# GregDMeyer/dynamite

Measured on AMD Instinct MI355X. Metric: matrix-free H|psi> Gamplitudes/s, random-field Heisenberg, higher is better.
Workload: dtype f64 (complex128)

## Files before the change

dynamite_amd/_lib.py:

```python
import ctypes as C
import os

import numpy as np

from . import build as _build

_HERE = os.path.dirname(os.path.abspath(__file__))

i64p = C.POINTER(C.c_int64)
f64p = C.POINTER(C.c_double)
vp = C.c_void_p


class Subspace(C.Structure):
    _fields_ = [("type", C.c_int32), ("L", C.c_int64), ("space", C.c_int64), ("k", C.c_int64),
                ("ld_nchoosek", C.c_int64), ("nchoosek", i64p), ("dim", C.c_int64),
                ("state_map", i64p), ("rmap_indices", i64p), ("rmap_states", i64p), ("vec_swizzle", C.c_int32),
                ("site_perm", C.POINTER(C.c_int8))]


class Partition(C.Structure):
    _fields_ = [("rank", C.c_int32), ("nranks", C.c_int32)]


MULT_FN = C.CFUNCTYPE(C.c_int, vp, vp, vp)
REDUCE_FN = C.CFUNCTYPE(C.c_int, vp, f64p, C.c_int)


class Hooks(C.Structure):
    _fields_ = [("ctx", vp), ("mult", MULT_FN), ("allreduce_sum", REDUCE_FN),
                ("allreduce_max", REDUCE_FN)]


class SolverStats(C.Structure):
    _fields_ = [("reason", C.c_int32), ("its", C.c_int32), ("matvecs", C.c_int32),
                ("nconv", C.c_int32), ("err_est", C.c_double)]


MAXSEG, MAXBSEG, MAXR = 4, 8, 16


LP_COUNT = 9
LP_NAMES = ["tile_real_k0", "tile_real", "tile_cplx", "tile_kvar_real", "tile_kvar_cplx", "gather_real",
            "gather_kvar_real", "gather_cplx", "gather_kvar_cplx"]
LP_KVAR, LP_CPLX, LP_GATHER = (3, 4, 6, 8), (2, 4, 7, 8), (5, 6, 7, 8)


class DevQuad(C.Structure):
    _fields_ = [("mask_tile", C.c_uint32), ("mask_loc", C.c_uint32), ("src", C.c_uint32),
                ("nslots", C.c_uint32), ("sign_tile", C.c_uint32 * 4), ("sign_ext", C.c_uint64 * 4),
                ("coeff", C.c_double * 4)]


class DevPass(C.Structure):
    _fields_ = [("nseg", C.c_int32), ("seg_off", C.c_int32 * MAXSEG), ("seg_len", C.c_int32 * MAXSEG),
                ("seg_pos", C.c_int32 * MAXSEG), ("nbseg", C.c_int32), ("bseg_off", C.c_int32 * MAXBSEG),
                ("bseg_len", C.c_int32 * MAXBSEG), ("bseg_pos", C.c_int32 * MAXBSEG),
                ("sign_base", C.c_uint64), ("accumulate", C.c_int32), ("need_tile", C.c_int32),
                ("has_diag", C.c_int32), ("cache_policy", C.c_int32), ("dext_begin", C.c_uint32), ("dext_end", C.c_uint32),
                ("dbucket", C.c_uint32 * (MAXR + 1)), ("loop", C.c_uint32 * (LP_COUNT + 1)),
                ("nquads", C.c_int32), ("n_eff", C.c_int32), ("quads", vp), ("dot_out", vp), ("zinit", vp), ("zscale", C.c_double), ("zinit2", vp), ("z2re", C.c_double), ("z2im", C.c_double),
                ("tile_bits", C.c_int32), ("log_rows", C.c_int32),
                ("swz_shift", C.c_int32), ("swz_xor_y", C.c_uint32), ("swz_xor_src", C.c_uint32), ("block_offset", C.c_uint32),
                ("pos_tmask", C.c_uint32), ("dtile", vp), ("tabs", vp), ("tabvals", vp), ("tab_loop", C.c_uint32 * 3),
                ("pad_tab", C.c_uint32), ("gbucket", C.c_uint32 * (MAXR + 1)), ("pad_g", C.c_uint32)]


class DevTab(C.Structure):
    _fields_ = [("mask_tile", C.c_uint32), ("mask_loc", C.c_uint32), ("src", C.c_uint32), ("first", C.c_uint32),
                ("z_tile", C.c_uint32), ("flags", C.c_uint32), ("tpos", C.c_uint32), ("twid", C.c_uint32),
                ("epos", C.c_uint32), ("ewid", C.c_uint32), ("z_ext", C.c_uint64), ("ik", C.c_uint64),
                ("ksign", C.c_uint32), ("nbits", C.c_uint32)]


class Xfer(C.Structure):
    _fields_ = [("partner", C.c_int32), ("pass_id", C.c_int32), ("offset", C.c_int64), ("count", C.c_int64)]


MAT_DEFAULT, MAT_FORCE_GATHER, MAT_USE_GLDS, MAT_HOST_ONLY = 0, 1, 2, 4
MAT_REAL_PACKED = 16
EXCHANGE_AUTO, EXCHANGE_PARTNER, EXCHANGE_TRANSPOSE = 0, 1, 2
PHASE_ALL, PHASE_EXCHANGE, PHASE_COMPUTE = 0, 1, 2
MAT_AMIN_SHIFT = 8
WHICH = {"lowest": 0, "highest": 1, "exterior": 2, "target": 3}
CONVERGED_TOL, CONVERGED_ITS, DIVERGED_ITS, DIVERGED_BREAKDOWN, DIVERGED_SYMMETRY_LOST = 1, 2, -1, -2, -3

SIGNATURES = {
    "dnm_last_error": (C.c_char_p, []),
    "dnm_version": (C.c_int, []),
    "dnm_device_count": (C.c_int, [C.POINTER(C.c_int)]),
    "dnm_set_device": (C.c_int, [C.c_int]),
    "dnm_malloc": (C.c_int, [C.POINTER(vp), C.c_size_t]),
    "dnm_free": (C.c_int, [vp]),
    "dnm_memcpy_h2d": (C.c_int, [vp, vp, C.c_size_t, vp]),
    "dnm_memcpy_d2h": (C.c_int, [vp, vp, C.c_size_t, vp]),
    "dnm_stream_synchronize": (C.c_int, [vp]),
    "dnm_subspace_dim": (C.c_int, [C.POINTER(Subspace), i64p]),
    "dnm_idx_to_state": (C.c_int, [C.POINTER(Subspace), C.c_int64, i64p, i64p]),
    "dnm_state_to_idx": (C.c_int, [C.POINTER(Subspace), C.c_int64, i64p, i64p]),
    "dnm_mat_create": (C.c_int, [C.c_int64, i64p, i64p, i64p, f64p, C.POINTER(Subspace),
                                 C.POINTER(Subspace), C.c_int, C.c_int, C.POINTER(Partition),
                                 C.POINTER(vp)]),
    "dnm_check_conserves": (C.c_int, [C.c_int64, i64p, i64p, i64p, f64p, C.POINTER(Subspace),
                                      C.POINTER(Subspace), C.c_int, C.POINTER(C.c_int), vp]),
    "dnm_reduced_density_matrix": (C.c_int, [vp, C.POINTER(Subspace), C.c_int, i64p, vp, vp]),
    "dnm_rdm_sector_plan": (C.c_int, [C.POINTER(Subspace), C.c_int, i64p, C.c_int, C.POINTER(C.c_int),
                                      C.POINTER(C.c_int32), i64p, i64p, C.POINTER(C.c_size_t)]),
    "dnm_rdm_sector_blocks": (C.c_int, [vp, C.POINTER(Subspace), C.c_int, i64p, C.c_int, C.c_int,
                                        C.POINTER(C.c_int32), C.POINTER(vp), vp]),
    "dnm_vec_set_random_swz": (C.c_int, [vp, C.c_int64, C.c_uint64, C.c_int64, C.c_int, vp]),
    "dnm_vec_swizzle_copy": (C.c_int, [vp, vp, C.c_int64, C.c_int, vp]),
    "dnm_vec_unpack_real": (C.c_int, [vp, vp, C.c_int64, C.c_int, C.c_int, vp]),
    "dnm_vec_layout_unpack_real": (C.c_int, [C.POINTER(Subspace), C.POINTER(Partition), vp, vp, vp]),
    "dnm_vec_layout_size": (C.c_int, [C.POINTER(Subspace), C.POINTER(C.c_int64)]),
    "dnm_vec_layout_partition": (C.c_int, [C.POINTER(Subspace), C.c_int, C.c_int, i64p, i64p, i64p, i64p]),
    "dnm_vec_layout_blocks": (C.c_int, [C.POINTER(Subspace), C.c_int64, i64p, i64p, i64p]),
    "dnm_vec_layout_copy": (C.c_int, [C.POINTER(Subspace), C.POINTER(Partition), vp, vp, C.c_int, vp]),
    "dnm_vec_layout_copy_f64": (C.c_int, [C.POINTER(Subspace), C.POINTER(Partition), vp, vp, C.c_int, vp]),
    "dnm_vec_layout_zero_padding": (C.c_int, [C.POINTER(Subspace), C.POINTER(Partition), vp, vp]),
    "dnm_vec_layout_positions": (C.c_int, [C.POINTER(Subspace), C.POINTER(Partition), C.c_int64, vp, vp, vp]),
    "dnm_vec_layout_positions_host": (C.c_int, [C.POINTER(Subspace), C.POINTER(Partition), C.c_int64, i64p, i64p]),
    "dnm_vec_layout_set_random": (C.c_int, [C.POINTER(Subspace), C.POINTER(Partition), vp, C.c_uint64, vp]),
    "dnm_mat_layouts": (C.c_int, [vp, C.POINTER(C.c_int), C.POINTER(C.c_int)]),
    "dnm_mat_window_split": (C.c_int, [vp, C.POINTER(C.c_int)]),
    "dnm_mat_mult_local_part": (C.c_int, [vp, vp, vp, C.c_int, C.c_int, vp]),
    "dnm_mat_local_part_bits": (C.c_int, [vp, C.POINTER(C.c_int), C.POINTER(C.c_int)]),
    "dnm_mat_mult_window_local": (C.c_int, [vp, vp, vp, vp]),
    "dnm_mat_mult_window_remote": (C.c_int, [vp, vp, C.c_int64, C.c_int64, vp, vp]),
    "dnm_mat_window_local_rows": (C.c_int, [vp, C.c_int64, C.c_int64, C.c_int, C.c_int, C.POINTER(C.c_int64), C.POINTER(C.c_int), vp]),
    "dnm_mat_mult_window_rows": (C.c_int, [vp, vp, C.c_int64, C.c_int64, vp, C.c_int64, C.c_int64, vp]),
    "dnm_mat_destroy": (C.c_int, [vp]),
    "dnm_mat_sizes": (C.c_int, [vp, i64p, i64p, i64p, i64p]),
    "dnm_mat_precompute_diagonal": (C.c_int, [vp, vp]),
    "dnm_mat_get_diagonal": (C.c_int, [vp, f64p, vp]),
    "dnm_mat_mult": (C.c_int, [vp, vp, vp, vp]),
    "dnm_mat_norm_inf": (C.c_int, [vp, f64p, vp]),
    "dnm_mat_set_norm": (C.c_int, [vp, C.c_double]),
    "dnm_mat_plan_describe": (C.c_int, [vp, C.c_char_p, C.c_size_t]),
    "dnm_mat_plan_launches": (C.c_int, [vp, C.POINTER(C.c_int)]),
    "dnm_mat_plan_counts": (C.c_int, [vp] + [C.POINTER(C.c_int)] * 6),
    "dnm_mat_export_dtile": (C.c_int, [vp, C.c_int, C.c_int, f64p, C.c_int64]),
    "dnm_mat_export_tabs": (C.c_int, [vp, C.c_int, C.c_int, vp, C.c_size_t, C.c_int, C.POINTER(C.c_int), f64p, C.c_int64, i64p]),
    "dnm_mat_export_pass": (C.c_int, [vp, C.c_int, C.c_int, vp, C.c_size_t, vp, C.c_size_t, C.c_int,
                                      C.POINTER(C.c_int)]),
    "dnm_mat_ownership": (C.c_int, [vp, i64p, i64p]),
    "dnm_mat_column_window": (C.c_int, [vp, i64p, i64p, vp]),
    "dnm_mat_column_chunks": (C.c_int, [vp, C.c_int, C.POINTER(C.c_uint8), C.c_int64, vp]),
    "dnm_mat_mult_window": (C.c_int, [vp, vp, C.c_int64, C.c_int64, vp, vp]),
    "dnm_mat_exchange_plan": (C.c_int, [vp, C.POINTER(C.c_int), C.POINTER(Xfer), C.POINTER(C.c_int),
                                        C.POINTER(Xfer)]),
    "dnm_mat_mult_dot": (C.c_int, [vp, vp, vp, f64p, vp]),
    "dnm_mat_mult_lanczos": (C.c_int, [vp, vp, vp, vp, C.c_double, f64p, vp]),
    "dnm_mat_mult_local": (C.c_int, [vp, vp, vp, vp]),
    "dnm_mat_mult_remote": (C.c_int, [vp, C.c_int32, vp, vp, vp]),
    "dnm_vec_set": (C.c_int, [vp, C.c_int64, C.c_double, C.c_double, vp]),
    "dnm_vec_copy": (C.c_int, [vp, vp, C.c_int64, vp]),
    "dnm_vec_scale": (C.c_int, [vp, C.c_int64, C.c_double, C.c_double, vp]),
    "dnm_vec_axpby": (C.c_int, [vp, vp, C.c_int64, C.c_double, C.c_double, C.c_double, C.c_double, vp]),
    "dnm_vec_dot": (C.c_int, [vp, vp, C.c_int64, f64p, vp]),
    "dnm_vec_norm2": (C.c_int, [vp, C.c_int64, f64p, vp]),
    "dnm_vec_set_random": (C.c_int, [vp, C.c_int64, C.c_uint64, C.c_int64, vp]),
    "dnm_vec_mdot": (C.c_int, [vp, C.c_int64, C.c_int, vp, C.c_int64, f64p, vp]),
    "dnm_vec_maxpy": (C.c_int, [vp, vp, C.c_int64, C.c_int, C.c_int64, f64p, vp]),
    "dnm_vec_basis_update": (C.c_int, [vp, C.c_int64, C.c_int, C.c_int, C.c_int64, f64p, vp]),
    "dnm_workspace_bytes": (C.c_int, [C.POINTER(C.c_size_t)]),
    "dnm_release_workspace": (C.c_int, []),
    "dnm_mat_is_real_packed": (C.c_int, [C.c_void_p, C.POINTER(C.c_int)]),
    "dnm_comm_unique_id": (C.c_int, [C.c_void_p]),
    "dnm_comm_create": (C.c_int, [C.c_void_p, C.c_int, C.c_int, C.POINTER(C.c_void_p)]),
    "dnm_comm_destroy": (C.c_int, [C.c_void_p]),
    "dnm_comm_forget": (C.c_int, [C.c_void_p, C.c_void_p]),
    "dnm_comm_loopback": (C.c_int, [C.c_void_p, C.c_int, C.c_int, C.POINTER(C.c_void_p), C.POINTER(C.c_void_p)]),
    "dnm_comm_allreduce": (C.c_int, [C.c_void_p, C.POINTER(C.c_double), C.c_int, C.c_int]),
    "dnm_mat_mult_partitioned": (C.c_int, [C.c_void_p, C.c_void_p, C.c_void_p, C.c_void_p, C.c_void_p]),
    "dnm_mat_column_ranges": (C.c_int, [C.c_void_p, C.c_int64, C.POINTER(C.c_int64), C.POINTER(C.c_int64)]),
    "dnm_comm_prepare": (C.c_int, [C.c_void_p, C.c_void_p, C.c_void_p]),
    "dnm_comm_set_phase": (C.c_int, [C.c_void_p, C.c_int]),
    "dnm_mat_set_exchange": (C.c_int, [C.c_void_p, C.c_int, C.POINTER(C.c_int)]),
    "dnm_mat_operator": (C.c_int, [C.c_void_p, i64p, i64p, i64p, i64p, i64p, f64p]),
    "dnm_mat_exchange_parts": (C.c_int, [C.c_void_p, C.POINTER(C.c_void_p), C.POINTER(C.c_void_p), C.POINTER(C.c_int)]),
    "dnm_comm_hooks": (C.c_int, [C.c_void_p, C.c_void_p, C.c_void_p, C.POINTER(Hooks)]),
    "dnm_sc_choose_site_perm": (C.c_int, [C.c_int, C.c_int, C.c_int, C.c_int64, i64p, C.c_int, C.POINTER(C.c_int8),
                                          C.POINTER(C.c_int32)]),
    "dnm_workspace_reserve": (C.c_int, [C.c_size_t, C.c_void_p]),
    "dnm_expm_chebyshev": (C.c_int, [vp, vp, vp, C.c_int64, C.c_double, C.c_double, C.POINTER(Hooks),
                                     C.POINTER(SolverStats), vp]),
    "dnm_mat_mult_sub": (C.c_int, [vp, vp, vp, vp, C.c_double, vp]),
    "dnm_mat_fuses_init": (C.c_int, [vp]),
    "dnm_mat_mult_sub2": (C.c_int, [vp, vp, vp, vp, C.c_double, vp, C.c_double, C.c_double, vp]),
    "dnm_expm_multiply": (C.c_int, [vp, vp, vp, C.c_int64, C.c_double, C.c_double, C.c_double, C.c_int,
                                    C.c_int, C.c_size_t, C.POINTER(Hooks), C.POINTER(SolverStats), vp]),
    "dnm_eigsolve": (C.c_int, [vp, C.c_int64, C.c_int, C.c_int, C.c_double, C.c_int, C.c_int,
                               C.c_uint64, C.POINTER(Hooks), C.c_int, f64p, vp,
                               C.POINTER(SolverStats), vp]),
    "dnm_eigsolve_interior": (C.c_int, [vp, C.c_int64, C.c_int, C.c_double, C.c_double, C.c_int, C.c_int,
                                        C.c_uint64, C.POINTER(Hooks), C.c_int, f64p, vp,
                                        C.POINTER(SolverStats), vp]),
    "dnm_interior_filter_plan": (C.c_int, [C.c_double, C.c_double, C.c_double, C.c_double, C.c_double,
                                           C.POINTER(C.c_int), f64p, f64p]),
}


class BackendError(RuntimeError):
    """Raised when a C-ABI call returns non-zero (the reference raises petsc4py.Error)."""


_lib = None


def lib():
    global _lib
    if _lib is None:
        import torch
        path = _build.build()
        import os
        if os.environ.get("DNM_EXPERIMENTAL") == "1":
            path = os.environ.get("DNM_LIB", path)
        L = C.CDLL(path)
        for name, (res, args) in SIGNATURES.items():
            fn = getattr(L, name)
            fn.restype = res
            fn.argtypes = args
        _lib = L
    return _lib


def check(rc):
    if rc != 0:
        raise BackendError(lib().dnm_last_error().decode())


def p64(a):
    return a.ctypes.data_as(i64p)


def pf64(a):
    return a.ctypes.data_as(f64p)


def device_count():
    n = C.c_int(0)
    lib().dnm_device_count(C.byref(n))
    return n.value
```

dynamite_amd/csrc/kernels.h:

```cpp
#pragma once

#include <vector>

#include "plan.h"
#include "subspace.h"

namespace dnm {

struct DevMsc {
  int32_t nmasks;
  const int64_t *masks;
  const int64_t *mask_offsets;
  const int64_t *signs;
  const double *real_coeffs;
};

bool tile_config_supported(int B, int logR);

int launch_tile_pass(const DevPass &P, int B, int logR, bool glds, int n_loc,
                     const void *x, void *y, const void *xr, hipStream_t st, unsigned nparts = 1);

struct ColMark {
  uint8_t *map = nullptr;
  int32_t shift = 0;
  int64_t first = 0;
};
int gather_num_blocks(int64_t M);
int gather_rows_per_block();
int launch_gather_matvec(const DevMsc &msc, const SubView &left, const SubView &right,
                         int64_t M, const double *diag, const void *x, void *y,
                         hipStream_t st, int64_t row0 = 0, int64_t win_start = 0, int xswz = -1,
                         int64_t *colrange = nullptr, ColMark mark = ColMark());

struct ScMask {
  int32_t fast;
  int32_t lo;
  double up_re, up_im, dn_re, dn_im;
  int32_t pair, hi, dead, pad;
};
std::vector<ScMask> sc_masks(const std::vector<int64_t> &masks, const std::vector<int64_t> &mask_offsets,
                             const std::vector<int64_t> &signs, const std::vector<double> &rcoef, int L = 0,
                             bool xparity = false);

struct ScLow {
  const uint16_t *tab;
  int32_t off[18];
};
int sc_num_blocks(int64_t M);
int sc_rows_per_block();
int launch_sc_matvec(const DevMsc &msc, const ScMask *scm, const ScLow &low, const SubView &sub, int64_t M, int64_t row0,
                     int64_t win_start, const double *diag, const void *xw, void *y, int64_t *colrange,
                     hipStream_t st, ColMark mark = ColMark());

struct ScBlock {
  const uint16_t *lowtab;
  int32_t off[18];
  int32_t lb;
  int32_t swizzle;
  int64_t h_first, h_last;
  const uint32_t *perm;
  int64_t nperm;
};
bool sc_block_supported(int lb);
int sc_block_max_masks();
int64_t sc_block_grid(const ScBlock &blk);
int launch_sc_block(const DevMsc &msc, const ScMask *scm, const ScBlock &blk, const SubView &sub, int64_t M, int64_t row0,
                    int64_t win_start, int64_t win_len, const double *diag, const void *xw, void *y,
                    hipStream_t st, const void *zinit = nullptr, double zscale = 0.0, double *dot_out = nullptr,
                    const void *zinit2 = nullptr, double z2re = 0.0, double z2im = 0.0);

int launch_diag(const DevMsc &msc, const SubView &sub, int64_t M, int64_t row0, double *diag, hipStream_t st);

int norm_num_blocks(int64_t M);
int launch_norm(const DevMsc &msc, const SubView &left, const SubView &right, int64_t M,
                int64_t row0, double *block_max, hipStream_t st);

int launch_conserves(const DevMsc &msc, const double *coeffs_im, const SubView &left, const SubView &right,
                     int64_t N, int *bad, hipStream_t st);

struct RdmGeom {
  int32_t k, L;
  int32_t nseg_keep, nseg_tr;
  int8_t klen[33], kpos[33];
  int8_t tlen[33], tpos[33];
};
void rdm_plan(const RdmGeom &geo, int *logtm, int *ntiles, int *nsplit, int64_t *chunks_per_split,
              size_t *partial_bytes);
int launch_rdm(const void *x, const SubView &sub, const RdmGeom &geo, void *partial, void *rho, hipStream_t st);
size_t rdm_partial_bytes(int64_t nsplit, int64_t nelem);
int rdm_sum_slices(void *partial, int64_t nelem, int *nsplit, void **level, hipStream_t st);

struct RdmSectorBlock {
  int32_t n, m;
  int64_t dim, traced;
  int64_t per_slice;
  void *out;
};
struct RdmSectorTile {
  int32_t blk, ti, tj, pad;
};
int rdm_sector_plan(int nblocks, RdmSectorBlock *blocks, int64_t *ntiles, int *nsplit, size_t *table_bytes,
                    size_t *partial_bytes);
int launch_rdm_sector(const void *x, const SubView &sub, const RdmGeom &geo, bool contig, int xparity_sector,
                      int nblocks, const RdmSectorBlock *blocks, int64_t ntiles, int nsplit, size_t table_bytes,
                      void *scratch, hipStream_t st);

int vk_set(void *x, int64_t n, double re, double im, hipStream_t st);
int vk_copy(void *y, const void *x, int64_t n, hipStream_t st);
int vk_scale(void *x, int64_t n, double re, double im, hipStream_t st);
int vk_axpby(void *y, const void *x, int64_t n, double are, double aim, double bre, double bim,
             hipStream_t st);
int vk_random(void *x, int64_t n, uint64_t seed, int64_t offset, hipStream_t st, int swz = 0);
int vk_swizzle_copy(void *dst, const void *src, int64_t n, int swz, hipStream_t st);
int vk_unpack_real(void *dst, const void *src, int64_t n_packed, int swz_src, int swz_dst, hipStream_t st);
int vk_mdot_blocks(int64_t n);
int vk_sweep_blocks(int64_t n);
size_t vk_sweep_scratch(int64_t n, int ncols);
int vk_mdot(const void *V, int64_t ldv, int nv, const void *w, int64_t n, double *partials_dev,
            hipStream_t st);
int vk_maxpy(void *w, const void *V, int64_t ldv, int nv, int64_t n, const double *c_dev,
             hipStream_t st);
int vk_basis_update(void *V, int64_t ldv, int nin, int nout, int64_t n, const double *S_dev,
                    hipStream_t st);
int vk_lanczos_update(void *p, const void *v, const void *u, int64_t n, double are, double aim, double b,
                      double scale, double *partials_dev, hipStream_t st);
int vk_lanczos_dot(void *y, const void *z, const void *x, int64_t n, double b, double *partials_dev,
                   hipStream_t st,
                   double yscale = 1.0);
size_t vk_reduce_scratch(int ncols);
int vk_reduce_partials(const double *partials, int nblocks, int ncols, double *out, hipStream_t st, double *tmp = nullptr);
int vk_norm2_partials(const void *x, int64_t n, double *partials_dev, hipStream_t st);

}
```

dynamite_amd/csrc/mat.cpp:

```cpp
#include "mat.h"
#include "vec_api.h"
#include "row_fused.h"

#include <algorithm>
#include <cstring>

namespace dnm {

static thread_local std::string g_err;

void set_error(const char *fmt, ...) {
  char buf[1024];
  va_list ap;
  va_start(ap, fmt);
  vsnprintf(buf, sizeof(buf), fmt, ap);
  va_end(ap);
  g_err = buf;
}

int DevBuf::alloc(size_t nbytes) {
  release();
  if (nbytes == 0) nbytes = 16;
  DNM_HIP(hipMalloc(&p, nbytes));
  bytes = nbytes;
// ... 75 lines not shown
      ++bucket[(size_t)(st >> host.bucket_shift) + 1];
    }
    if (sorted) {
      for (int64_t b = 0; b < nb; ++b) bucket[(size_t)b + 1] += bucket[(size_t)b];
      host.bucket = bucket.data();
    } else {
      bucket.clear();
      host.bucket = nullptr;
    }
  }
  host.dim = sub_dim(host);
  dev = host;
  dev.nchoosek = nullptr;
  dev.state_map = dev.rmap_indices = dev.rmap_states = nullptr;
  dev.bucket = nullptr;
  if (want_device) {
    if (!nck.empty()) {
      DNM_TRY(d_nck.upload(nck.data(), nck.size() * 8));
      dev.nchoosek = (const int64_t *)d_nck.p;
    }
    if (!smap.empty()) {
      DNM_TRY(d_smap.upload(smap.data(), smap.size() * 8));
      DNM_TRY(d_rstates.upload(rstates.data(), rstates.size() * 8));
      dev.state_map = (const int64_t *)d_smap.p;
      dev.rmap_states = (const int64_t *)d_rstates.p;
      if (!rind.empty()) {
        DNM_TRY(d_rind.upload(rind.data(), rind.size() * 8));
        dev.rmap_indices = (const int64_t *)d_rind.p;
      }
      if (!bucket.empty()) {
        DNM_TRY(d_bucket.upload(bucket.data(), bucket.size() * 8));
        dev.bucket = (const int64_t *)d_bucket.p;
      }
    }
  }
  return 0;
}

static int build_opform(const dnm_mat &A, OpForm *op) {
  const SubView &l = A.left.host, &r = A.right.host;
  const bool par = l.type == DNM_PARITY;
  const int n = par ? l.L - 1 : l.L;
  op->n = n;
  op->masks.clear();
  const uint64_t ones = n >= 64 ? ~0ull : (((uint64_t)1 << n) - 1);
  for (size_t mi = 0; mi < A.masks.size(); ++mi) {
    const uint64_t mask = (uint64_t)A.masks[mi];
    if (par && (parity64(mask) != (l.space ^ r.space))) continue;
    RowMask rm;
    rm.mask = par ? (mask >> 1) : mask;
    for (int64_t t = A.mask_offsets[mi]; t < A.mask_offsets[mi + 1]; ++t) {
      const uint64_t sg = (uint64_t)A.signs[t];
      RowTerm rt;
      rt.is_imag = parity64(mask & sg);
      double c = A.real_coeffs[t];
      uint64_t s2 = sg;
      if (par) {
        s2 = sg >> 1;
        if (sg & 1) {
          s2 ^= ones;
          if (r.space) c = -c;
        }
      }
      if (parity64(rm.mask & s2)) c = -c;
      rt.sign = s2;
      rt.coeff = c;
      rm.terms.push_back(rt);
    }
    if (rm.mask == 0) {
      RowMask im;
      im.mask = 0;
      im.zero_mask_offdiag = true;
      std::vector<RowTerm> re;
      for (const RowTerm &t : rm.terms) (t.is_imag ? im.terms : re).push_back(t);
      rm.terms.swap(re);
      if (!im.terms.empty()) op->masks.push_back(std::move(im));
      if (rm.terms.empty()) continue;
    }
    op->masks.push_back(std::move(rm));
  }
  std::stable_sort(op->masks.begin(), op->masks.end(),
            [](const RowMask &a, const RowMask &b) { return a.mask < b.mask; });
  return 0;
}

static uint32_t compress_to_tile(uint64_t bits, const PassSpec &ps) {
  uint32_t out = 0;
  int off = 0;
  for (int j = 0; j < ps.nseg; ++j) {
    uint64_t seg = (bits >> ps.seg_pos[j]) & (((uint64_t)1 << ps.seg_len[j]) - 1);
    out |= (uint32_t)seg << off;
    off += ps.seg_len[j];
  }
  return out;
}

static int pack_opform(OpForm *op) {
  DNM_CHECK(op->n >= 2, "real-packed form needs at least two index bits");
  std::vector<RowMask> out;
  for (const RowMask &rm : op->masks) {
    for (const RowTerm &t : rm.terms) DNM_CHECK(!t.is_imag, "operator has an imaginary matrix element: no real-packed form");
    DNM_CHECK(!rm.zero_mask_offdiag, "operator has an imaginary matrix element: no real-packed form");
    RowMask lanes;
    lanes.mask = rm.mask >> 1;
    lanes.pack_flip = (rm.mask & 1) != 0;
    if (rm.mask == 0) {
      RowMask diag;
      diag.mask = 0;
      lanes.zero_mask_offdiag = true;
      for (const RowTerm &t : rm.terms) {
        if (!(t.sign & 1)) { diag.terms.push_back({t.sign >> 1, t.coeff, 0}); continue; }
        lanes.terms.push_back({t.sign >> 1, t.coeff, 0});
        lanes.terms.push_back({t.sign >> 1, -t.coeff, 1});
      }
      if (!diag.terms.empty()) out.push_back(std::move(diag));
      if (!lanes.terms.empty()) out.push_back(std::move(lanes));
      continue;
    }
    lanes.zero_mask_offdiag = lanes.mask == 0;
    bool same = !lanes.pack_flip;
    for (const RowTerm &t : rm.terms) same = same && !(t.sign & 1);
    for (const RowTerm &t : rm.terms) {
      lanes.terms.push_back({t.sign >> 1, t.coeff, 0});
      if (!same) lanes.terms.push_back({t.sign >> 1, (t.sign & 1) ? -t.coeff : t.coeff, 1});
    }
    out.push_back(std::move(lanes));
  }
  std::stable_sort(out.begin(), out.end(), [](const RowMask &a, const RowMask &b) {
    if (a.mask != b.mask) return a.mask < b.mask;
    return (int)a.zero_mask_offdiag < (int)b.zero_mask_offdiag;
  });
  op->masks.swap(out);
  op->n -= 1;
  op->packed = true;
  return 0;
}

static bool table_form(const OpForm &op, const RowMask &m, std::vector<uint64_t> *zs) {
  const char *tabs_env = knob("DNM_TAB_RECORDS");
  if (tabs_env && tabs_env[0] == '0') return false;
  const int nb = __builtin_popcountll(m.mask);
  if (op.packed || m.pack_flip || nb < 1 || nb > MAXTABBITS || m.terms.size() < 5) return false;
  size_t nre = 0, nim = 0;
  zs->clear();
  for (const RowTerm &t : m.terms) {
    (t.is_imag ? nim : nre)++;
    const uint64_t z = t.sign & ~m.mask;
    if (std::find(zs->begin(), zs->end(), z) == zs->end()) zs->push_back(z);
  }
  const size_t nq = std::max((nre + 1) / 2, (nim + 1) / 2);
  return nq >= 2 && zs->size() * 45 < nq * 76;
}

static int build_pass(const dnm_mat &A, const PassSpec &ps, PassOnDevice *out) {
  const OpForm &op = A.op;
  const Plan &pl = A.plan;
  const int B = ps.B;
  int logR = ps.logR ? ps.logR : pl.cfg.logR;
  {
    std::vector<uint64_t> zs;
    bool any = false;
    for (int idx : ps.tile_masks) any = any || table_form(op, op.masks[idx], &zs);
    for (int idx : ps.gather_masks) any = any || table_form(op, op.masks[idx], &zs);
    int want = 3;
    if (const char *e = knob("DNM_TAB_LOG_ROWS")) want = atoi(e);
    if (any && want > logR && tile_config_supported(B, want)) logR = want;
  }
  {
    auto top_thread_pos = [&](int lr) {
      int c = 0, top = -1;
      for (int j = 0; j < ps.nseg; ++j)
        for (int i = 0; i < ps.seg_len[j]; ++i, ++c)
          if (c < B - lr) top = std::max(top, ps.seg_pos[j] + i);
      return top;
    };
    while (top_thread_pos(logR) >= 28 && tile_config_supported(B, logR + 1)) ++logR;
  }
  const int lognt = B - logR, R = 1 << logR;
  const int n_eff = ps.n_eff ? ps.n_eff : pl.n_loc;
  const uint64_t tb = ps.tile_bits();
  DevPass &d = out->desc;
  memset(&d, 0, sizeof(d));
  d.nseg = ps.nseg;
  int off = 0;
  for (int j = 0; j < ps.nseg; ++j) {
    d.seg_off[j] = off;
    d.seg_len[j] = ps.seg_len[j];
    d.seg_pos[j] = ps.seg_pos[j];
    off += ps.seg_len[j];
  }
  DNM_CHECK(off == B, "internal: tile segments do not add up to B");
  {
    std::vector<int> order;
    uint64_t gb = ps.glen ? ((((uint64_t)1 << ps.glen) - 1) << ps.gpos) : 0;
    std::vector<int> rest;
    for (int pos = 0; pos < n_eff; ++pos)
      if (!((tb >> pos) & 1) && !((gb >> pos) & 1)) rest.push_back(pos);
    size_t nsel = ps.glen ? std::min<size_t>(3, rest.size()) : 0;
    for (size_t i = 0; i < nsel; ++i) order.push_back(rest[i]);
    for (int pos = ps.gpos; pos < ps.gpos + ps.glen; ++pos) order.push_back(pos);
    for (size_t i = nsel; i < rest.size(); ++i) order.push_back(rest[i]);
    if (const char *e = knob("DNM_ORDER_WINDOW")) {
      if (ps.nseg > 1 && ps.partner < 0) {
        std::vector<int> o;
        for (const char *q = e; *q;) {
          o.push_back(atoi(q));
          while (*q && *q != ',') ++q;
          if (*q == ',') ++q;
        }
        std::vector<int> a = o, b2 = order;
        std::sort(a.begin(), a.end());
        std::sort(b2.begin(), b2.end());
        DNM_CHECK(a == b2, "DNM_ORDER_WINDOW is not a permutation of the block bits");
        order = o;
      }
    }
    DNM_CHECK((int)order.size() == n_eff - B, "internal: block bits do not add up");
    int nb = 0;
    for (size_t i = 0; i < order.size();) {
      size_t j = i + 1;
      while (j < order.size() && order[j] == order[j - 1] + 1) ++j;
      DNM_CHECK(nb < MAXBSEG, "internal: too many block segments");
      d.bseg_off[nb] = (int32_t)i;
      d.bseg_len[nb] = (int32_t)(j - i);
      d.bseg_pos[nb] = order[i];
      ++nb;
      i = j;
    }
    d.nbseg = nb;
  }
  d.sign_base = ((uint64_t)pl.rank << pl.n_loc) | ps.sign_extra;
  d.n_eff = n_eff;
  d.tile_bits = B;
  d.log_rows = logR;
  DNM_CHECK(tile_config_supported(B, logR), "unsupported tile configuration B=%d logR=%d", B, logR);
  d.accumulate = ps.accumulate ? 1 : 0;
  d.has_diag = 0;
  d.cache_policy = pl.cfg.cache_policy | (op.packed ? 256 : 0);
  {
    const int S = pl.cfg.swz;
    DNM_CHECK(S == 0 || (S >= 5 && S <= 24), "swizzle shift %d out of range", S);
    d.swz_shift = S;
    auto sw = [S](uint64_t v) -> uint32_t {
      return S ? (uint32_t)(((v >> S) & (((uint64_t)1 << (S - 4)) - 1)) << 4) : 0u;
    };
    d.swz_xor_y = sw((uint64_t)ps.y_off);
    d.swz_xor_src = sw((uint64_t)ps.src_off);
    uint64_t tm = 0;
    int c = 0;
    for (int j = 0; j < ps.nseg; ++j)
      for (int i = 0; i < ps.seg_len[j]; ++i, ++c)
        if (c < lognt) tm |= ((uint64_t)1 << (ps.seg_pos[j] + i)) | sw((uint64_t)1 << (ps.seg_pos[j] + i));
    DNM_CHECK((tm >> 28) == 0, "internal: thread bits of the tile above bit 27 (tile %llx, %d rows per thread)",
              (unsigned long long)tb, R);
    d.pos_tmask = (uint32_t)tm;
  }

  std::vector<DevQuad> quads;
  auto empty_quad = [&]() {
    DevQuad q;
    memset(&q, 0, sizeof(q));
    return q;
  };
  auto set_slot = [&](DevQuad &q, int slot, const RowTerm &t) {
    q.sign_ext[slot] = t.sign & ~tb;
    q.sign_tile[slot] = compress_to_tile(t.sign & tb, ps);
    q.coeff[slot] = t.coeff;
  };
  auto push_diag_list = [&](const std::vector<RowTerm> &lst) {
    for (size_t i = 0; i < lst.size(); i += 4) {
      DevQuad q = empty_quad();
      for (size_t j = i; j < lst.size() && j < i + 4; ++j) {
        set_slot(q, (int)(j - i), lst[j]);
        q.nslots = (uint32_t)(j - i + 1);
      }
      quads.push_back(q);
    }
  };

  if (ps.has_diag) {
    const RowMask *dm = nullptr;
    for (const RowMask &m : op.masks) if (m.mask == 0 && !m.zero_mask_offdiag) dm = &m;
    if (dm) {
      d.has_diag = 1;
      std::vector<RowTerm> lst;
      for (const RowTerm &t : dm->terms)
        if (compress_to_tile(t.sign & tb, ps) == 0) lst.push_back(t);
      d.dext_begin = (uint32_t)quads.size();
      push_diag_list(lst);
      d.dext_end = (uint32_t)quads.size();
      const char *dte = knob("DNM_DIAG_TABLE");
      const bool use_table = !(dte && dte[0] == '0') && B <= 13;
      if (use_table) out->h_dtile.assign((size_t)1 << B, 0.0);
      std::vector<std::pair<uint32_t, std::vector<RowTerm>>> groups;
      {
        const char *dge = knob("DNM_DIAG_GROUPS");
        const bool grouping = !(dge && dge[0] == '0') && !op.packed && !(A.flags & DNM_MAT_USE_GLDS);
        std::vector<std::pair<uint32_t, std::vector<RowTerm>>> all;
        if (grouping)
          for (const RowTerm &t : dm->terms) {
            const uint32_t st = compress_to_tile(t.sign & tb, ps);
            if (st == 0 || (t.sign & ~tb) == 0) continue;
            auto it = std::find_if(all.begin(), all.end(), [&](const auto &g) { return g.first == st; });
            if (it == all.end()) { all.push_back({st, {}}); it = all.end() - 1; }
            it->second.push_back(t);
          }
        std::stable_sort(all.begin(), all.end(), [](const auto &a, const auto &b) { return a.second.size() > b.second.size(); });
        for (auto &g : all)
          if (g.second.size() >= 3 && groups.size() < MAXDGROUPS) groups.push_back(std::move(g));
      }
      auto grouped = [&](uint32_t st) {
        return std::any_of(groups.begin(), groups.end(), [&](const auto &g) { return g.first == st; });
      };
      for (int j = 0; j < R; ++j) {
        lst.clear();
        for (const RowTerm &t : dm->terms) {
          uint32_t st = compress_to_tile(t.sign & tb, ps);
          if (st == 0 || (int)(st >> lognt) != j) continue;
          if (use_table && (t.sign & ~tb) == 0) {
            for (uint32_t tc = 0; tc < (1u << B); ++tc)
              out->h_dtile[tc] += (__builtin_popcount(tc & st) & 1) ? -t.coeff : t.coeff;
          } else if ((t.sign & ~tb) != 0 && grouped(st)) {
            continue;
          } else {
            lst.push_back(t);
          }
        }
        d.dbucket[j] = (uint32_t)quads.size();
        push_diag_list(lst);
      }
      for (int j = R; j <= MAXR; ++j) d.dbucket[j] = (uint32_t)quads.size();
      std::vector<std::pair<uint32_t, uint32_t>> where(groups.size());
      for (size_t g = 0; g < groups.size(); ++g) {
        std::vector<RowTerm> outside = groups[g].second;
        for (RowTerm &t : outside) t.sign &= ~tb;
        where[g].first = (uint32_t)quads.size();
        push_diag_list(outside);
        where[g].second = (uint32_t)quads.size() - where[g].first;
      }
      for (int j = 0; j < R; ++j) {
        d.gbucket[j] = (uint32_t)quads.size();
        for (size_t g = 0; g < groups.size(); ++g) {
          if ((int)(groups[g].first >> lognt) != j) continue;
          DevQuad q = empty_quad();
          q.sign_tile[0] = groups[g].first;
          q.mask_loc = where[g].first;
          q.src = where[g].second;
          q.nslots = 1;
          quads.push_back(q);
        }
      }
      for (int j = R; j <= MAXR; ++j) d.gbucket[j] = (uint32_t)quads.size();
    }
  }

  struct Rec { int loop; DevQuad q; };
  std::vector<Rec> recs;
  std::vector<DevTab> tabs_tile, tabs_gather;
  std::vector<double> tabvals;
  auto push_tabs = [&](const RowMask &m, uint64_t mloc, bool gather, int src) -> bool {
    std::vector<uint64_t> zs;
    if (!table_form(op, m, &zs)) return false;
    const int nb = __builtin_popcountll(m.mask);
    int pb[MAXTABBITS];
    for (int q = 0, pos = 0; pos < 64; ++pos)
      if ((m.mask >> pos) & 1ull) pb[q++] = pos;
    for (uint64_t z : zs) {
      DevTab T;
      memset(&T, 0, sizeof(T));
      T.mask_tile = compress_to_tile(mloc & tb, ps);
      T.mask_loc = (uint32_t)mloc;
      T.src = (uint32_t)src;
      T.nbits = (uint32_t)nb;
      const uint32_t zt = compress_to_tile(z & tb, ps);
      T.z_tile = zt & ((1u << lognt) - 1u);
      T.z_ext = z & ~tb;
      T.first = (uint32_t)(tabvals.size() / 2);
      for (int k = 0; k < R; ++k)
        if (__builtin_popcount((uint32_t)k & (zt >> lognt)) & 1) T.ksign |= 1u << k;
      for (int q = 0; q < nb; ++q) {
        if ((tb >> pb[q]) & 1ull) {
          const int tpos = __builtin_ctz(compress_to_tile((uint64_t)1 << pb[q], ps));
          if (tpos < lognt) {
            T.tpos |= (uint32_t)tpos << (8 * q);
            T.twid |= 1u << (8 * q);
          } else {
            T.flags |= 1u;
            for (int k = 0; k < R; ++k)
              if ((k >> (tpos - lognt)) & 1) T.ik |= (uint64_t)1 << (4 * k + q);
          }
        } else {
          T.epos |= (uint32_t)pb[q] << (8 * q);
          T.ewid |= 1u << (8 * q);
        }
      }
      for (int j = 0; j < (1 << nb); ++j) {
        uint64_t rowbits = 0;
        for (int q = 0; q < nb; ++q)
          if ((j >> q) & 1) rowbits |= (uint64_t)1 << pb[q];
        double re = 0.0, im = 0.0;
        for (const RowTerm &t : m.terms) {
          if ((t.sign & ~m.mask) != z) continue;
          const double c = (__builtin_popcountll(rowbits & t.sign & m.mask) & 1) ? -t.coeff : t.coeff;
          (t.is_imag ? im : re) += c;
        }
        tabvals.push_back(re);
        tabvals.push_back(im);
      }
      if (z == zs.back()) T.flags |= 2u;
      (gather ? tabs_gather : tabs_tile).push_back(T);
    }
    return true;
  };
  auto push_mask = [&](int idx, bool gather, int src) {
    const RowMask &m = op.masks[idx];
    const uint64_t mloc = m.mask & (((uint64_t)1 << n_eff) - 1);
    if (!gather) DNM_CHECK((mloc & ~tb) == 0, "internal: tile mask leaves the tile");
    if (push_tabs(m, mloc, gather, src)) return 0;
    std::vector<const RowTerm *> re, im;
    for (const RowTerm &t : m.terms) (t.is_imag ? im : re).push_back(&t);
    size_t ir = 0, ii = 0;
    while (ir < re.size() || ii < im.size()) {
      DevQuad q = empty_quad();
      q.mask_tile = compress_to_tile(mloc & tb, ps);
      q.mask_loc = (uint32_t)mloc;
      q.src = (uint32_t)src;
      q.nslots = m.pack_flip ? 1u : 0u;
      bool kvar = false, cplx = false;
      for (int s = 0; s < 2 && ir < re.size(); ++s, ++ir) {
        set_slot(q, s, *re[ir]);
        kvar |= (q.sign_tile[s] >> lognt) != 0;
      }
      for (int s = 2; s < 4 && ii < im.size(); ++s, ++ii) {
        set_slot(q, s, *im[ii]);
        kvar |= (q.sign_tile[s] >> lognt) != 0;
        cplx = true;
      }
      int loop;
      if (gather) loop = kvar ? (cplx ? LP_GATHER_KVAR_CPLX : LP_GATHER_KVAR_REAL) : (cplx ? LP_GATHER_CPLX : LP_GATHER_REAL);
      else if (kvar) loop = cplx ? LP_TILE_KVAR_CPLX : LP_TILE_KVAR_REAL;
      else if (cplx) loop = LP_TILE_CPLX;
      else loop = (q.mask_tile >> lognt) == 0 ? LP_TILE_REAL_K0 : LP_TILE_REAL;
      recs.push_back({loop, q});
    }
    return 0;
  };
  for (int idx : ps.tile_masks) DNM_TRY(push_mask(idx, false, 0));
  for (size_t i = 0; i < ps.gather_masks.size(); ++i)
    DNM_TRY(push_mask(ps.gather_masks[i], true, ps.gather_src[i]));
  for (int lp = 0; lp < LP_COUNT; ++lp) {
    d.loop[lp] = (uint32_t)quads.size();
    for (const Rec &r : recs) if (r.loop == lp) quads.push_back(r.q);
  }
  d.loop[LP_COUNT] = (uint32_t)quads.size();

  d.nquads = (int32_t)quads.size();
  d.need_tile = (d.has_diag || !ps.tile_masks.empty()) ? 1 : 0;
  d.tab_loop[0] = 0;
  d.tab_loop[1] = (uint32_t)tabs_tile.size();
  d.tab_loop[2] = (uint32_t)(tabs_tile.size() + tabs_gather.size());
  out->h_tabs = tabs_tile;
  out->h_tabs.insert(out->h_tabs.end(), tabs_gather.begin(), tabs_gather.end());
  out->h_tabvals = tabvals;
  d.tabs = nullptr;
  d.tabvals = nullptr;
  if (!out->h_tabs.empty() && !A.host_only) {
    DNM_TRY(out->tabs.upload(out->h_tabs.data(), out->h_tabs.size() * sizeof(DevTab)));
    DNM_TRY(out->tabvals.upload(out->h_tabvals.data(), out->h_tabvals.size() * sizeof(double)));
    d.tabs = (const DevTab *)out->tabs.p;
    d.tabvals = (const double *)out->tabvals.p;
  }
  out->h_quads = quads;
  if (!A.host_only) DNM_TRY(out->quads.upload(quads.data(), quads.size() * sizeof(DevQuad)));
  d.quads = (const DevQuad *)out->quads.p;
  d.dtile = nullptr;
  if (!out->h_dtile.empty() && !A.host_only) {
    DNM_TRY(out->dtile.upload(out->h_dtile.data(), out->h_dtile.size() * sizeof(double)));
    d.dtile = (const double *)out->dtile.p;
  }
  out->partner = ps.partner;
  out->n_eff = n_eff;
  out->y_off = ps.y_off;
  out->src_off = ps.src_off;
  return 0;
}

static hipStream_t S(void *stream) { return (hipStream_t)stream; }

static int launch_pass(const dnm_mat *A, const PassOnDevice &p, const DevPass &d, const void *x, void *y,
                       const void *xr, hipStream_t st, unsigned nparts = 1) {
  return launch_tile_pass(d, d.tile_bits, d.log_rows, (A->flags & DNM_MAT_USE_GLDS) != 0, p.n_eff, x, y, xr, st, nparts);
}

static size_t pass_dot_partials(const dnm_mat *, const PassOnDevice &p) {
  return (size_t)1 << (p.n_eff - p.desc.tile_bits);
}

}

using namespace dnm;

namespace dnm {
std::vector<ScMask> sc_masks(const std::vector<int64_t> &masks, const std::vector<int64_t> &mask_offsets,
                             const std::vector<int64_t> &signs, const std::vector<double> &rcoef, int L, bool xparity) {
  std::vector<ScMask> scm(masks.size());
  for (size_t mi = 0; mi < masks.size(); ++mi) {
    ScMask &e = scm[mi];
    memset(&e, 0, sizeof(e));
    const uint64_t mask = (uint64_t)masks[mi];
    e.dead = __builtin_popcountll(mask) & 1;
    if (xparity && L >= 3 && __builtin_popcountll(mask) == L - 2 && !((mask >> (L - 1)) & 1ull)) {
      const uint64_t miss = ~mask & ((((uint64_t)1 << (L - 1)) - 1));
      const int i = __builtin_ctzll(miss);
      const uint64_t pairbits = ((uint64_t)1 << i) | ((uint64_t)1 << (L - 1));
      bool local = true;
      for (int64_t t = mask_offsets[mi]; t < mask_offsets[mi + 1]; ++t)
        if ((uint64_t)signs[t] & ~pairbits) local = false;
      if (!local) continue;
      e.pair = 2;
      e.lo = i;
      e.hi = L - 1;
      for (int64_t t = mask_offsets[mi]; t < mask_offsets[mi + 1]; ++t) {
        const double c = (((uint64_t)signs[t] >> i) & 1) ? -rcoef[t] : rcoef[t];
        e.up_re += c;
        e.dn_re += c;
      }
      continue;
    }
    if (__builtin_popcountll(mask) != 2) continue;
    const int lo = __builtin_ctzll(mask), hi = 63 - __builtin_clzll(mask);
    bool local = true;
    for (int64_t t = mask_offsets[mi]; t < mask_offsets[mi + 1]; ++t)
      if ((uint64_t)signs[t] & ~mask) local = false;
    if (!local) continue;
    e.pair = 1;
    e.fast = hi == lo + 1;
    e.lo = lo;
    e.hi = hi;
    for (int64_t t = mask_offsets[mi]; t < mask_offsets[mi + 1]; ++t) {
      const uint64_t sg = (uint64_t)signs[t];
      const double rc = rcoef[t];
      const bool imag = parity64(mask & sg);
      const double up = ((sg >> hi) & 1) ? -rc : rc;
      const double dn = ((sg >> lo) & 1) ? -rc : rc;
      (imag ? e.up_im : e.up_re) += up;
      (imag ? e.dn_im : e.dn_re) += dn;
    }
  }
  return scm;
}
}

extern "C" {

const char *dnm_last_error(void) { return g_err.c_str(); }
int dnm_version(void) { return 100; }

int dnm_device_count(int *count) {
  DNM_CHECK(count, "null pointer");
  hipError_t e = hipGetDeviceCount(count);
  if (e != hipSuccess) { *count = 0; (void)hipGetLastError(); }
  return 0;
}
int dnm_set_device(int device) { DNM_HIP(hipSetDevice(device)); return 0; }
int dnm_malloc(void **dptr, size_t bytes) { DNM_HIP(hipMalloc(dptr, bytes ? bytes : 16)); return 0; }
int dnm_free(void *dptr) { DNM_HIP(hipFree(dptr)); return 0; }
int dnm_memcpy_h2d(void *dst, const void *src, size_t bytes, void *stream) {
  DNM_HIP(hipMemcpyAsync(dst, src, bytes, hipMemcpyHostToDevice, S(stream)));
  DNM_HIP(hipStreamSynchronize(S(stream)));
  return 0;
}
int dnm_memcpy_d2h(void *dst, const void *src, size_t bytes, void *stream) {
  DNM_HIP(hipMemcpyAsync(dst, src, bytes, hipMemcpyDeviceToHost, S(stream)));
  DNM_HIP(hipStreamSynchronize(S(stream)));
  return 0;
}
int dnm_stream_synchronize(void *stream) { DNM_HIP(hipStreamSynchronize(S(stream))); return 0; }

int dnm_subspace_dim(const dnm_subspace *s, int64_t *dim) {
  SubView v{};
  DNM_TRY(view_from_c(s, &v));
  *dim = sub_dim(v);
  return 0;
}

int dnm_idx_to_state(const dnm_subspace *s, int64_t n, const int64_t *idxs, int64_t *states) {
  SubView v{};
  DNM_TRY(view_from_c(s, &v));
  const int64_t dim = sub_dim(v);
  for (int64_t i = 0; i < n; ++i) {
    DNM_CHECK(idxs[i] >= 0 && idxs[i] < dim, "index %lld out of bounds for subspace of dimension %lld",
              (long long)idxs[i], (long long)dim);
    states[i] = sub_i2s(idxs[i], v);
  }
  return 0;
}

int dnm_state_to_idx(const dnm_subspace *s, int64_t n, const int64_t *states, int64_t *idxs) {
  SubView v{};
  DNM_TRY(view_from_c(s, &v));
  for (int64_t i = 0; i < n; ++i) idxs[i] = sub_s2i(states[i], v);
  return 0;
}

int dnm_check_conserves(int64_t nmasks, const int64_t *masks, const int64_t *mask_offsets,
                        const int64_t *signs, const double *coeffs, const dnm_subspace *left,
                        const dnm_subspace *right, int xparity, int *result, void *stream) {
  DNM_CHECK(result && (nmasks == 0 || (masks && mask_offsets && signs && coeffs)), "null argument");
  SubOwned l, r;
  DNM_TRY(l.init(left, true));
  DNM_TRY(r.init(right, true));
  const int64_t nterms = nmasks ? mask_offsets[nmasks] : 0;
  std::vector<double> re(nterms), im(nterms);
  for (int64_t t = 0; t < nterms; ++t) { re[t] = coeffs[2 * t]; im[t] = coeffs[2 * t + 1]; }
  DevBuf dm, doff, ds, dre, dim_, dbad;
  DNM_TRY(dm.upload(masks, (size_t)nmasks * 8));
  DNM_TRY(doff.upload(mask_offsets, (size_t)(nmasks + 1) * 8));
  DNM_TRY(ds.upload(signs, (size_t)nterms * 8));
  DNM_TRY(dre.upload(re.data(), (size_t)nterms * 8));
  DNM_TRY(dim_.upload(im.data(), (size_t)nterms * 8));
  int zero = 0;
  DNM_TRY(dbad.upload(&zero, sizeof(int)));
  DevMsc msc{(int32_t)nmasks, (const int64_t *)dm.p, (const int64_t *)doff.p, (const int64_t *)ds.p,
             (const double *)dre.p};
  const int64_t ncols = xparity ? r.host.dim / 2 : r.host.dim;
  DNM_TRY(launch_conserves(msc, (const double *)dim_.p, l.dev, r.dev, ncols, (int *)dbad.p, S(stream)));
  int bad = 0;
  DNM_TRY(dnm_memcpy_d2h(&bad, dbad.p, sizeof(int), stream));
  *result = bad ? 0 : 1;
  return 0;
}

static DevBuf g_rdm_scratch;
}
namespace dnm {
int rdm_release_scratch() {
  g_rdm_scratch.release();
  return 0;
}
}
extern "C" {

static void rdm_geom(int L, int keep_size, const int64_t *keep, RdmGeom *out) {
  RdmGeom &geo = *out;
// ... 304 lines not shown
  if (lt == DNM_SPIN_CONSERVE && rt == DNM_SPIN_CONSERVE)
    scm = sc_masks(A->masks, A->mask_offsets, A->signs, A->real_coeffs, A->left.host.L, A->xparity);
  if (!A->host_only) {
  DNM_TRY(A->d_masks.upload(A->masks.data(), A->masks.size() * 8));
  DNM_TRY(A->d_offsets.upload(A->mask_offsets.data(), A->mask_offsets.size() * 8));
  DNM_TRY(A->d_signs.upload(A->signs.data(), A->signs.size() * 8));
  DNM_TRY(A->d_rcoeffs.upload(A->real_coeffs.data(), A->real_coeffs.size() * 8));
  A->dmsc.nmasks = (int32_t)nmasks;
  A->dmsc.masks = (const int64_t *)A->d_masks.p;
  A->dmsc.mask_offsets = (const int64_t *)A->d_offsets.p;
  A->dmsc.signs = (const int64_t *)A->d_signs.p;
  A->dmsc.real_coeffs = (const double *)A->d_rcoeffs.p;
  if (lt == DNM_SPIN_CONSERVE && rt == DNM_SPIN_CONSERVE) {
    A->sc_nfast = 0;
    for (const ScMask &e : scm) A->sc_nfast += e.fast ? 1 : 0;
    DNM_TRY(A->d_scmasks.upload(scm.data(), scm.size() * sizeof(ScMask)));
    std::vector<uint16_t> low(65536);
    int cnt[18] = {0};
    for (int v = 0; v < 65536; ++v) ++cnt[__builtin_popcount(v) + 1];
    for (int j = 0; j < 17; ++j) { cnt[j + 1] += cnt[j]; A->sclow.off[j] = cnt[j]; }
    A->sclow.off[17] = 65536;
    int fill[17];
    for (int j = 0; j < 17; ++j) fill[j] = A->sclow.off[j];
    for (int v = 0; v < 65536; ++v) low[fill[__builtin_popcount(v)]++] = (uint16_t)v;
    DNM_TRY(A->d_sclow.upload(low.data(), low.size() * sizeof(uint16_t)));
    A->sclow.tab = (const uint16_t *)A->d_sclow.p;
    if (!A->use_sc3) DNM_TRY(setup_sc_block(A.get()));
  }
  }
  if (A->use_sc3) {
    const SubView &h = A->left.host;
    const Sc3Layout *ly = sc3_get(h.L, h.k, sc3_code_a(h.sc3), sc3_code_w(h.sc3), !A->host_only, sc3_code_order(h.sc3));
    DNM_CHECK(ly, "could not build the SpinConserve vector layout");
    A->sc3.reset(new Sc3Mat());
    std::vector<uint32_t> Tb = sc3_partition(*ly, A->nranks);
    if (A->xparity) Tb = {0u, 1u << (ly->host.t - 1)};
    const bool want_real = (flags & DNM_MAT_REAL_PACKED) != 0;
    Sc3Perm P, Pr;
    DNM_CHECK(sc3_perm_make(left->site_perm, h.L, &P) && sc3_perm_make(right->site_perm, h.L, &Pr),
              "site_perm is not a permutation of the %d spins", h.L);
    DNM_CHECK(memcmp(P.to_int, Pr.to_int, sizeof P.to_int) == 0, "left and right vectors must share their site relabelling");
    DNM_CHECK(!P.on || A->nranks == 1, "a relabelled SpinConserve layout is not partitioned over ranks");
    DNM_CHECK(!A->xparity || P.to_int[h.L - 1] == h.L - 1, "XParity: the site relabelling must keep spin L-1 in place");
    A->sc3->perm = P;
    std::vector<int64_t> pmasks = A->masks, poffs = A->mask_offsets, psigns = A->signs;
    std::vector<double> pcoef = A->real_coeffs;
    if (P.on) {
      std::vector<int64_t> order((size_t)nmasks);
      std::vector<uint64_t> nm((size_t)nmasks);
      for (int64_t i = 0; i < nmasks; ++i) {
        order[(size_t)i] = i;
        nm[(size_t)i] = sc3_permute((uint64_t)A->masks[(size_t)i], P.to_int, h.L);
      }
      std::sort(order.begin(), order.end(), [&](int64_t x, int64_t y) { return nm[(size_t)x] < nm[(size_t)y]; });
      pmasks.clear(); psigns.clear(); pcoef.clear();
      poffs.assign(1, 0);
      for (int64_t q = 0; q < nmasks; ++q) {
        const int64_t i = order[(size_t)q];
        pmasks.push_back((int64_t)nm[(size_t)i]);
        for (int64_t t = A->mask_offsets[(size_t)i]; t < A->mask_offsets[(size_t)i + 1]; ++t) {
          psigns.push_back((int64_t)sc3_permute((uint64_t)A->signs[(size_t)t], P.to_int, h.L));
          pcoef.push_back(A->real_coeffs[(size_t)t]);
        }
        poffs.push_back((int64_t)psigns.size());
      }
      scm = sc_masks(pmasks, poffs, psigns, pcoef, h.L, A->xparity);
      if (!A->host_only) {
        DNM_TRY(A->d_pmasks.upload(pmasks.data(), pmasks.size() * 8));
        DNM_TRY(A->d_poffsets.upload(poffs.data(), poffs.size() * 8));
        DNM_TRY(A->d_psigns.upload(psigns.data(), psigns.size() * 8));
        DNM_TRY(A->d_prcoeffs.upload(pcoef.data(), pcoef.size() * 8));
      }
    }
    A->dmsc_sc3 = A->dmsc;
    if (P.on && !A->host_only) {
      A->dmsc_sc3.masks = (const int64_t *)A->d_pmasks.p;
      A->dmsc_sc3.mask_offsets = (const int64_t *)A->d_poffsets.p;
      A->dmsc_sc3.signs = (const int64_t *)A->d_psigns.p;
      A->dmsc_sc3.real_coeffs = (const double *)A->d_prcoeffs.p;
    }
    DNM_TRY(A->sc3->init(ly, pmasks, poffs, psigns, pcoef, scm, !A->host_only, Tb[A->rank],
                         Tb[A->rank + 1], want_real));
    if (const char *e = knob("DNM_SC3_TILED")) if (e[0] == '0') A->sc3->tiled = false;
    if (const char *e = knob("DNM_SC3_DIAG")) if (e[0] == 'c' && A->sc3->diag_mode == 2) A->sc3->diag_mode = 1;
    if (const char *e = knob("DNM_SC3_DIAG")) if (e[0] == 'n') A->sc3->diag_mode = 0;
    int64_t is, il, ns, nl;
    sc3_range(*ly, Tb[A->rank], Tb[A->rank + 1], &is, &il, &ns, &nl);
    A->m_local = A->n_local = il;
    A->rows_local = nl;
    A->row0 = ns;
    if (want_real) {
      DNM_CHECK(A->sc3->tiled && A->sc3->sym,
                "operator has an imaginary matrix element or is not a sum of pair hops: no real-packed form in this layout");
      A->real_packed = true;
      A->m_local = A->n_local = il / 2;
    }
  } else if (flags & DNM_MAT_REAL_PACKED) {
    DNM_CHECK(A->hypercube, "real-packed operators: Full / Parity pairs, or a SpinConserve pair in the internal layout");
  }

  if (A->hypercube) {
    DNM_TRY(build_opform(*A, &A->op));
    if (flags & DNM_MAT_REAL_PACKED) {
      DNM_CHECK(A->M == A->N, "real-packed operators: square");
      DNM_TRY(pack_opform(&A->op));
      A->real_packed = true;
      A->M /= 2; A->N /= 2; A->m_local /= 2; A->n_local /= 2;
    }
    if (A->xparity) {
      const uint64_t topbit = (uint64_t)1 << (A->op.n - 1);
      for (RowMask &rm : A->op.masks) {
        DNM_CHECK(!(rm.mask & topbit), "internal: XParity mask reaches the top index bit");
        for (RowTerm &t : rm.terms) t.sign &= ~topbit;
      }
      A->op.n -= 1;
    }
    PlanConfig cfg = plan_config_from_env();
    if (const int fa = (flags >> DNM_MAT_AMIN_SHIFT) & 0xff) cfg.amin = fa;
    DNM_CHECK(A->left.host.swz == A->right.host.swz, "left and right vectors of a Full/Parity pair must share a layout");
    cfg.swz = A->left.host.swz;
    if (cfg.logR < 0) {
      int nl = A->op.n;
      for (int r = A->nranks; r > 1; r >>= 1) --nl;
      cfg.logR = cfg.swz ? 2 : (nl >= 26 ? 4 : 3);
    }
    if (cfg.diag_last < 0) cfg.diag_last = cfg.swz ? 1 : 0;
    if (cfg.window_first < 0) {
      int nl = A->op.n;
      for (int r = A->nranks; r > 1; r >>= 1) --nl;
      cfg.window_first = (cfg.swz && nl >= 25) ? 1 : 0;
    }
    if (!tile_config_supported(cfg.B, cfg.logR)) {
      set_error("unsupported tile configuration B=%d logR=%d", cfg.B, cfg.logR);
      return 1;
    }
    DNM_TRY(make_plan(A->op, A->rank, A->nranks, cfg, &A->plan));
    if (flags & DNM_MAT_FORCE_GATHER) A->plan.use_tiled = false;
    DNM_CHECK(!A->real_packed || A->plan.use_tiled, "real-packed operators run on the tiled kernel only (vector too small)");
    if (A->nranks > 1 && !A->plan.use_tiled) {
      A->plan.remote.clear();
      A->plan.sends.clear();
    }
    if (A->plan.use_tiled) {
      for (const PassSpec &ps : A->plan.local) {
        std::unique_ptr<PassOnDevice> p(new PassOnDevice());
        DNM_TRY(build_pass(*A, ps, p.get()));
        A->local_passes.push_back(std::move(p));
      }
      for (const PassSpec &ps : A->plan.remote) {
        std::unique_ptr<PassOnDevice> p(new PassOnDevice());
        DNM_TRY(build_pass(*A, ps, p.get()));
        A->remote_passes.push_back(std::move(p));
      }
    }
  }
  *out = A.release();
  return 0;
}

int dnm_mat_destroy(dnm_mat *A) {
  delete A;
  return 0;
}

int dnm_mat_set_exchange(dnm_mat *A, int scheme, int *chosen) {
  DNM_CHECK(A && chosen, "null argument");
  DNM_CHECK(scheme == DNM_EXCHANGE_AUTO || scheme == DNM_EXCHANGE_PARTNER || scheme == DNM_EXCHANGE_TRANSPOSE,
            "unknown exchange scheme %d", scheme);
  delete A->tr_lo; delete A->tr_hi;
  A->tr_lo = A->tr_hi = nullptr;
  A->tr_f = -1;
  *chosen = DNM_EXCHANGE_PARTNER;
  const int P = A->nranks;
  if (scheme == DNM_EXCHANGE_PARTNER || P < 2 || (scheme == DNM_EXCHANGE_AUTO && P < 4)) return 0;
  const SubView &lh = A->left.host, &rh = A->right.host;
  if (!(A->hypercube && A->plan.use_tiled && !A->xparity && lh.type == rh.type && lh.L == rh.L &&
        (lh.type == DNM_FULL || lh.space == rh.space) && lh.swz == rh.swz))
    return 0;
  int p = 0;
  while ((1 << p) < P) ++p;
  const int shift = lh.type == DNM_PARITY ? 1 : 0;
  const int packed = A->real_packed ? 1 : 0;
  const int n = (int)lh.L - shift - p, f = n - 1 - p;
  if ((1 << p) != P || f < packed) return 0;
  if (lh.swz && f - packed < 2 * lh.swz - 4) return 0;
  const int fs = f + shift, ns = n + shift;
  const int64_t fld = P - 1;
  struct Term { int64_t m, s; double c; };
  std::vector<Term> lo, hi;
  for (size_t i = 0; i < A->masks.size(); ++i)
    for (int64_t t = A->mask_offsets[i]; t < A->mask_offsets[i + 1]; ++t) {
      const int64_t m = A->masks[i], s = A->signs[(size_t)t];
      if ((m >> ns) == 0) { lo.push_back({m, s, A->real_coeffs[(size_t)t]}); continue; }
      if ((m >> fs) & fld) return 0;
      auto swap = [&](int64_t v) {
        const int64_t d = ((v >> fs) ^ (v >> ns)) & fld;
        return v ^ (d << fs) ^ (d << ns);
      };
      hi.push_back({swap(m), swap(s), A->real_coeffs[(size_t)t]});
    }
  if (lo.empty() || hi.empty()) return 0;
  const int np = n - packed, fp = f - packed;
  dnm_subspace ld{}, rd{};
  ld.type = lh.type; ld.L = lh.L; ld.space = lh.space; ld.vec_swizzle = lh.swz;
  rd.type = rh.type; rd.L = rh.L; rd.space = rh.space; rd.vec_swizzle = rh.swz;
  const dnm_partition part{A->rank, A->nranks};
  dnm_mat *made[2] = {nullptr, nullptr};
  for (int which = 0; which < 2; ++which) {
    std::vector<Term> &T = which ? hi : lo;
    std::stable_sort(T.begin(), T.end(), [](const Term &a, const Term &b) { return a.m < b.m; });
    std::vector<int64_t> masks, offs, signs;
    std::vector<double> coeffs;
    for (size_t i = 0; i < T.size(); ++i) {
      if (i == 0 || T[i].m != T[i - 1].m) { masks.push_back(T[i].m); offs.push_back((int64_t)i); }
      signs.push_back(T[i].s);
      coeffs.push_back(T[i].c); coeffs.push_back(0.0);
    }
    offs.push_back((int64_t)T.size());
    int fl = A->flags & ~(0xff << DNM_MAT_AMIN_SHIFT);
    if (which == 1 && np - fp <= 8) {
      const char *tb = knob("DNM_TILE_BITS");
      const int a = (tb ? atoi(tb) : 12) - (np - fp);
      if (a >= 2 && a <= 9) fl |= a << DNM_MAT_AMIN_SHIFT;
    } else {
      fl |= A->flags & (0xff << DNM_MAT_AMIN_SHIFT);
    }
    int rc = dnm_mat_create((int64_t)masks.size(), masks.data(), offs.data(), signs.data(), coeffs.data(), &ld, &rd, 0, fl,
                            &part, &made[which]);
    int ns_ = 0, nr_ = 0;
    if (rc == 0) rc = dnm_mat_exchange_plan(made[which], &ns_, nullptr, &nr_, nullptr);
    if (rc == 0 && (ns_ || nr_)) { set_error("transposed exchange: a pass is not rank-local"); rc = 1; }
    if (rc == 0 && !(made[which]->hypercube && made[which]->plan.use_tiled)) {
      set_error("transposed exchange: a part of the operator has no tiled plan"); rc = 1;
    }
    if (rc != 0) { delete made[0]; delete made[1]; return rc; }
  }
  A->tr_lo = made[0];
  A->tr_hi = made[1];
  A->tr_f = fp;
  *chosen = DNM_EXCHANGE_TRANSPOSE;
  return 0;
}

int dnm_mat_operator(const dnm_mat *A, int64_t *nmasks, int64_t *nterms, int64_t *masks, int64_t *mask_offsets,
                     int64_t *signs, double *coeffs) {
  DNM_CHECK(A && nmasks && nterms, "null argument");
  *nmasks = (int64_t)A->masks.size();
  *nterms = (int64_t)A->signs.size();
  if (masks) std::copy(A->masks.begin(), A->masks.end(), masks);
  if (mask_offsets) std::copy(A->mask_offsets.begin(), A->mask_offsets.end(), mask_offsets);
  if (signs) std::copy(A->signs.begin(), A->signs.end(), signs);
  if (coeffs) std::copy(A->real_coeffs.begin(), A->real_coeffs.end(), coeffs);
  return 0;
}

int dnm_mat_exchange_parts(const dnm_mat *A, dnm_mat **lo, dnm_mat **hi, int *f) {
  DNM_CHECK(A && lo && hi && f, "null argument");
  *lo = A->tr_lo; *hi = A->tr_hi; *f = A->tr_f;
  return 0;
}

int dnm_mat_sizes(const dnm_mat *A, int64_t *M, int64_t *N, int64_t *m_local, int64_t *n_local) {
  DNM_CHECK(A, "null matrix");
  if (M) *M = A->M;
  if (N) *N = A->N;
  if (m_local) *m_local = A->m_local;
  if (n_local) *n_local = A->n_local;
  return 0;
}

int dnm_mat_layouts(const dnm_mat *A, int *left, int *right) {
  DNM_CHECK(A, "null matrix");
  if (left) *left = A->use_sc3 ? A->left.host.sc3 : A->left.host.swz;
  if (right) *right = A->use_sc3 ? A->right.host.sc3 : A->right.host.swz;
  return 0;
}

int dnm_mat_is_real_packed(const dnm_mat *A, int *packed) {
  DNM_CHECK(A && packed, "null argument");
  *packed = A->real_packed ? 1 : 0;
  return 0;
}

static int sc3_mult(dnm_mat *A, const void *x, void *y, const void *z, double b, const void *z2, double c_re, double c_im,
                    double *dot3_host, void *stream, int64_t win_start = -1, int phase = 0) {
  Sc3Call call;
  call.row0 = A->sc3->row0;
  call.win_start = win_start >= 0 ? win_start : A->sc3->row0;
  call.zinit = (const double2 *)z;
  call.zscale = b;
  call.zinit2 = (const double2 *)z2;
  call.z2re = c_re;
  call.z2im = c_im;
  const double *dg = A->have_diag ? (const double *)A->diag.p : nullptr;
  if (!dot3_host) return launch_sc3(*A->sc3, A->dmsc_sc3, call, dg, x, y, S(stream), phase);
  const size_t nwg = sc3_dot_partials(*A->sc3);
  double *part = nullptr;
  DNM_TRY(vec_scratch(((nwg + 1) * 3 + vk_reduce_scratch(3)) * sizeof(double), &part));
  call.dot_out = part;
  DNM_TRY(launch_sc3(*A->sc3, A->dmsc_sc3, call, dg, x, y, S(stream)));
  DNM_TRY(vk_reduce_partials(part, (int)nwg, 3, part + 3 * nwg, S(stream), part + 3 * nwg + 3));
  DNM_HIP(hipMemcpyAsync(dot3_host, part + 3 * nwg, 3 * sizeof(double), hipMemcpyDeviceToHost, S(stream)));
  DNM_HIP(hipStreamSynchronize(S(stream)));
  return 0;
}

// ... 430 lines not shown
  DNM_CHECK(A->use_sc3 && A->sc3->tiled, "this operator's window multiply does not split (dnm_mat_window_split)");
  int64_t lo, hi;
  DNM_TRY(dnm_mat_column_window(A, &lo, &hi, stream));
  DNM_CHECK(win_start <= lo && win_start + win_len > hi,
            "window [%lld, %lld) does not cover the positions [%lld, %lld] this rank reads", (long long)win_start,
            (long long)(win_start + win_len), (long long)lo, (long long)hi);
  return sc3_mult(A, x_window, y_local, nullptr, 0.0, nullptr, 0.0, 0.0, nullptr, stream,
                  A->real_packed ? 2 * win_start : win_start, 2);
}

int dnm_mat_exchange_plan(const dnm_mat *A, int *nsend, dnm_xfer *sends, int *nrecv, dnm_xfer *recvs) {
  DNM_CHECK(A && nsend && nrecv, "null argument");
  *nsend = (int)A->plan.sends.size();
  *nrecv = (int)A->remote_passes.size();
  if (sends)
    for (size_t i = 0; i < A->plan.sends.size(); ++i)
      sends[i] = {A->plan.sends[i].partner, -1, A->plan.sends[i].offset, A->plan.sends[i].count};
  if (recvs)
    for (size_t i = 0; i < A->remote_passes.size(); ++i) {
      const auto &p = A->remote_passes[i];
      recvs[i] = {p->partner, (int32_t)i, p->src_off, (int64_t)1 << p->n_eff};
    }
  return 0;
}

int dnm_mat_mult_remote(dnm_mat *A, int32_t recv_index, const void *x_recv, void *y, void *stream) {
  DNM_CHECK(A && x_recv && y, "null argument");
  DNM_CHECK(!A->host_only, "host-only handle cannot multiply");
  DNM_CHECK(recv_index >= 0 && recv_index < (int)A->remote_passes.size(), "rank %d has no receive %d", A->rank,
            recv_index);
  const auto &p = A->remote_passes[recv_index];
  return launch_pass(A, *p, p->desc, x_recv, (char *)y + (size_t)p->y_off * 16, x_recv, S(stream));
}

int dnm_mat_norm_inf(dnm_mat *A, double *nrm, void *stream) {
  DNM_CHECK(A && nrm, "null argument");
  DNM_CHECK(!A->host_only, "host-only handle has no device tables");
  if (A->nrm != -1.0) {
    *nrm = A->nrm;
    return 0;
  }
  const int nb = norm_num_blocks(A->rows_local);
  DNM_TRY(A->scratch.alloc((size_t)nb * sizeof(double)));
  DNM_TRY(launch_norm(A->dmsc, A->left.dev, A->right.dev, A->rows_local, A->row0,
                      (double *)A->scratch.p, S(stream)));
  std::vector<double> h(nb);
  DNM_TRY(dnm_memcpy_d2h(h.data(), A->scratch.p, (size_t)nb * sizeof(double), stream));
  double best = 0.0;
  for (double v : h) best = std::max(best, v);
  if (A->nranks == 1) A->nrm = best;
  *nrm = best;
  return 0;
}

int dnm_mat_set_norm(dnm_mat *A, double nrm) {
  DNM_CHECK(A, "null matrix");
  A->nrm = nrm;
  return 0;
}

int dnm_mat_plan_describe(const dnm_mat *A, char *buf, size_t buflen) {
  DNM_CHECK(A && buf && buflen, "null argument");
  std::string s;
  if (A->hypercube) s = A->plan.describe(A->op);
  else if (A->use_sc3) {
    const Sc3Tab &T = A->sc3->ly->host;
    char tmp[512];
    if (A->sc3->tiled && A->sc3->graph)
      snprintf(tmp, sizeof tmp, "SpinConserve two-pass kernels on a bond graph, internal layout [T %d | W %d | Lo %d]: "
               "window pass (%zu workgroups, %d hops in LDS, %d gathered) then lo pass (%zu workgroups, %d hops in LDS, "
               "%d gathered), diagonal %s, coefficients %s\n", T.t, T.w, T.a, A->sc3->permB.size(), A->sc3->op.nldsB,
               A->sc3->op.ngatB, A->sc3->permA.size() / 8, A->sc3->op.nldsA, A->sc3->op.ngatA,
               A->sc3->diag_mode == 2 ? "on the fly" : (A->sc3->diag_mode == 1 ? "cached" : "none"),
               A->sc3->sym ? "real symmetric" : "complex");
    else if (A->sc3->tiled)
      snprintf(tmp, sizeof tmp, "SpinConserve two-pass kernels, internal layout [T %d | W %d | Lo %d]: window pass (%zu "
               "workgroups, %d bonds in LDS, %d gathered) then lo pass (%zu workgroups, %d bonds in LDS, %d gathered), "
               "diagonal %s, coefficients %s\n", T.t, T.w, T.a, A->sc3->permB.size(), T.w - 1,
               __builtin_popcountll(A->sc3->op.bondsB), A->sc3->permA.size() / 8, T.a - 1,
               __builtin_popcountll(A->sc3->op.bondsA),
               A->sc3->diag_mode == 2 ? "on the fly" : (A->sc3->diag_mode == 1 ? "cached" : "none"),
               A->sc3->sym ? "real symmetric" : "complex");
    else
      snprintf(tmp, sizeof tmp, "SpinConserve row kernel, internal layout [T %d | W %d | Lo %d] (positions by table)\n",
               T.t, T.w, T.a);
    s = tmp;
  } else if (A->sc_pair)
    s = A->scblock.lb ? "SpinConserve kernel, block form (" + std::to_string(A->scblock.lb) +
                            " low bits per workgroup in LDS, high bonds as block runs)\n"
                      : std::string("SpinConserve kernel (one row per thread, incremental colex rank)\n");
  else s = A->nranks > 1 ? "generic row-gather kernel (rows split in index order, columns through a window)\n"
                         : "generic row-gather kernel (non-hypercube subspace pair)\n";
  if (A->hypercube && !A->plan.use_tiled) s += "generic row-gather kernel in use\n";
  if (A->hypercube && A->plan.use_tiled) {
    size_t ntab = 0, nquad = 0;
    for (const auto &p : A->local_passes) { ntab += p->h_tabs.size(); nquad += p->desc.loop[LP_COUNT] - p->desc.loop[0]; }
    for (const auto &p : A->remote_passes) { ntab += p->h_tabs.size(); nquad += p->desc.loop[LP_COUNT] - p->desc.loop[0]; }
    if (ntab) s += "table records: " + std::to_string(ntab) + " (beside " + std::to_string(nquad) + " records of four terms)\n";
  }
  snprintf(buf, buflen, "%s", s.c_str());
  return 0;
}

int dnm_mat_export_pass(const dnm_mat *A, int remote, int idx, void *desc_out, size_t desc_bytes,
                        void *quads_out, size_t quad_bytes, int max_quads, int *nquads) {
  DNM_CHECK(A && nquads, "null argument");
  const auto &v = remote ? A->remote_passes : A->local_passes;
  DNM_CHECK(idx >= 0 && idx < (int)v.size(), "pass index out of range");
  const PassOnDevice &p = *v[idx];
  *nquads = (int)p.h_quads.size();
  if (desc_out) {
    DNM_CHECK(desc_bytes == sizeof(DevPass), "DevPass size mismatch (%zu vs %zu)", desc_bytes, sizeof(DevPass));
    memcpy(desc_out, &p.desc, sizeof(DevPass));
  }
  if (quads_out) {
    DNM_CHECK(quad_bytes == sizeof(DevQuad), "DevQuad size mismatch (%zu vs %zu)", quad_bytes, sizeof(DevQuad));
    DNM_CHECK(max_quads >= *nquads, "record buffer too small");
    if (!p.h_quads.empty()) memcpy(quads_out, p.h_quads.data(), p.h_quads.size() * sizeof(DevQuad));
  }
  return 0;
}

int dnm_mat_export_tabs(const dnm_mat *A, int remote, int idx, void *tabs_out, size_t tab_bytes, int max_tabs, int *ntabs,
                        double *vals_out, int64_t max_vals, int64_t *nvals) {
  DNM_CHECK(A && ntabs && nvals, "null argument");
  const auto &v = remote ? A->remote_passes : A->local_passes;
  DNM_CHECK(idx >= 0 && idx < (int)v.size(), "pass index out of range");
  const PassOnDevice &p = *v[idx];
  *ntabs = (int)p.h_tabs.size();
  *nvals = (int64_t)p.h_tabvals.size();
  if (tabs_out && !p.h_tabs.empty()) {
    DNM_CHECK(tab_bytes == sizeof(DevTab), "DevTab size mismatch (%zu vs %zu)", tab_bytes, sizeof(DevTab));
    DNM_CHECK(max_tabs >= *ntabs, "record buffer too small");
    memcpy(tabs_out, p.h_tabs.data(), p.h_tabs.size() * sizeof(DevTab));
  }
  if (vals_out && !p.h_tabvals.empty()) {
    DNM_CHECK(max_vals >= *nvals, "table buffer too small");
    memcpy(vals_out, p.h_tabvals.data(), p.h_tabvals.size() * sizeof(double));
  }
  return 0;
}

int dnm_mat_export_dtile(const dnm_mat *A, int remote, int idx, double *out, int64_t n) {
  DNM_CHECK(A && out, "null argument");
  const auto &v = remote ? A->remote_passes : A->local_passes;
  DNM_CHECK(idx >= 0 && idx < (int)v.size(), "pass index out of range");
  const PassOnDevice &p = *v[idx];
  DNM_CHECK((int64_t)p.h_dtile.size() == n, "the pass has %zu tabulated diagonal entries, not %lld", p.h_dtile.size(),
            (long long)n);
  memcpy(out, p.h_dtile.data(), p.h_dtile.size() * sizeof(double));
  return 0;
}

int dnm_mat_plan_counts(const dnm_mat *A, int *n_local_passes, int *n_remote_passes, int *tiled,
                        int *B, int *logR, int *n_loc) {
  DNM_CHECK(A, "null matrix");
  if (n_local_passes) *n_local_passes = (int)A->local_passes.size();
  if (n_remote_passes) *n_remote_passes = (int)A->remote_passes.size();
  if (tiled) *tiled = (A->hypercube && A->plan.use_tiled) ? 1 : 0;
  if (B) *B = A->plan.cfg.B;
  if (logR) *logR = A->plan.cfg.logR;
  if (n_loc) *n_loc = A->plan.n_loc;
  return 0;
}

int dnm_mat_plan_launches(const dnm_mat *A, int *n) {
  DNM_CHECK(A && n, "null argument");
  *n = (A->hypercube && A->plan.use_tiled) ? (int)A->local_passes.size() : 1;
  return 0;
}

}

dnm_mat::~dnm_mat() {
  delete tr_lo;
  delete tr_hi;
}
```

dynamite_amd/csrc/mat.h:

```cpp
#pragma once

#include <memory>
#include <vector>

#include "kernels.h"
#include "plan.h"
#include "sc3.h"
#include "subspace.h"

namespace dnm {

struct DevBuf {
  void *p = nullptr;
  size_t bytes = 0;
  DevBuf() = default;
  DevBuf(const DevBuf &) = delete;
  DevBuf &operator=(const DevBuf &) = delete;
  ~DevBuf() { release(); }
  int alloc(size_t nbytes);
  int upload(const void *host, size_t nbytes);
  void release();
};

struct SubOwned {
  SubView host{};
  SubView dev{};
  std::vector<int64_t> nck, smap, rind, rstates, bucket;
  DevBuf d_nck, d_smap, d_rind, d_rstates, d_bucket;
  int init(const dnm_subspace *s, bool want_device);
};

struct PassOnDevice {
  DevPass desc{};
  std::vector<DevQuad> h_quads;
  DevBuf quads;
  std::vector<double> h_dtile;
  DevBuf dtile;
  std::vector<DevTab> h_tabs;
  std::vector<double> h_tabvals;
  DevBuf tabs, tabvals;
  int partner = -1;
  int n_eff = 0;
  int64_t y_off = 0, src_off = 0;
};

int rdm_release_scratch();

}

struct dnm_mat {
  std::vector<int64_t> masks, mask_offsets, signs;
  std::vector<double> real_coeffs;
  dnm::SubOwned left, right;
  int64_t M = 0, N = 0, m_local = 0, n_local = 0;
  int64_t row0 = 0;
  bool sc_pair = false;
  bool use_sc3 = false;
  std::unique_ptr<dnm::Sc3Mat> sc3;
  int64_t rows_local = 0;
  int64_t win_min = 0, win_max = -1;
  int rank = 0, nranks = 1;
  int flags = 0;
  bool xparity = false;
  bool host_only = false;

  bool hypercube = false;
  bool real_packed = false;
  dnm::OpForm op;
  dnm::Plan plan;
  std::vector<std::unique_ptr<dnm::PassOnDevice>> local_passes, remote_passes;

  dnm::DevBuf d_masks, d_offsets, d_signs, d_rcoeffs;
  dnm::DevMsc dmsc{};
  dnm::DevBuf d_pmasks, d_poffsets, d_psigns, d_prcoeffs;
  dnm::DevMsc dmsc_sc3{};
  dnm::DevBuf d_sclow;
  dnm::ScLow sclow{};
  dnm::DevBuf d_scblock;
  dnm::DevBuf d_scperm;
  dnm::ScBlock scblock{};
  bool row_fuse = true;
  int sc_nfast = 0;
  double expm_tstep = 0.0;
  int expm_m = 0;
  int expm_bound = 0;
  dnm::DevBuf d_scmasks;

  dnm_mat *tr_lo = nullptr, *tr_hi = nullptr;
  int tr_f = -1;
  ~dnm_mat();

  dnm::DevBuf diag;
  bool have_diag = false;
  double nrm = -1.0;
  dnm::DevBuf scratch;
};
```

dynamite_amd/csrc/matvec_kernels.hip:

```cpp
#include <algorithm>
#include <cstdint>
#include <cstdlib>

#include "kernels.h"

namespace dnm {

typedef double2 c128;

#define GLOBAL_AS __attribute__((address_space(1)))
#define LDS_AS __attribute__((address_space(3)))

typedef double d2v __attribute__((ext_vector_type(2)));

typedef const __attribute__((address_space(4))) DevQuad CQuad;

__device__ __forceinline__ void store_through(c128 *p, double re, double im) {
  d2v v = {re, im};
  asm volatile("global_store_dwordx4 %0, %1, off sc1\n\ts_nop 1" ::"v"(p), "v"(v) : "memory");
}
__device__ __forceinline__ void store_streaming(c128 *p, double re, double im) {
  d2v v = {re, im};
  __builtin_nontemporal_store(v, reinterpret_cast<d2v *>(p));
}
__device__ __forceinline__ c128 load_streaming(const c128 *p) {
  d2v v = __builtin_nontemporal_load(reinterpret_cast<const d2v *>(p));
  return make_double2(v.x, v.y);
}

#ifdef DNM_PHASE_TIMING
__device__ unsigned long long *g_phase_buf = nullptr;
#define DNM_PH(i, waitvm)                                                                                  \
  do {                                                                                                     \
    if (waitvm) asm volatile("s_waitcnt vmcnt(0)" ::: "memory");                                           \
    if (g_phase_buf && threadIdx.x == 0)                                                                   \
      g_phase_buf[((size_t)(P.accumulate ? gridDim.x : 0) + blockIdx.x) * 8 + (i)] = wall_clock64();        \
    asm volatile("" ::: "memory");                                                                         \
  } while (0)
#else
#define DNM_PH(i, waitvm)
#endif

#ifndef DNM_XP_PRIO
#define DNM_XP_PRIO 1
#endif
#if DNM_XP_PRIO == 1
#define DNM_PRIO_MEM() asm volatile("s_setprio 3")
#define DNM_PRIO_LDS() asm volatile("s_setprio 0")
#else
#define DNM_PRIO_MEM()
#define DNM_PRIO_LDS()
#endif

__device__ __forceinline__ double flip_sign(double c, uint32_t parity_bit) {
  int hi = __double2hiint(c) ^ (int)(parity_bit << 31);
  return __hiloint2double(hi, __double2loint(c));
}

__device__ __forceinline__ double slot_amp(CQuad &q, int j, uint32_t tt, uint64_t sbase) {
  uint32_t p = (uint32_t)(__popc(tt & q.sign_tile[j]) + __popcll(sbase & q.sign_ext[j])) & 1u;
  return flip_sign(q.coeff[j], p);
}

template <int MAXS>
__device__ __forceinline__ uint32_t deposit(uint32_t v, int nseg, const int32_t *off,
                                            const int32_t *len, const int32_t *pos) {
  uint32_t r = 0;
#pragma unroll
  for (int j = 0; j < MAXS; ++j)
    if (j < nseg) r |= ((v >> off[j]) & ((1u << len[j]) - 1u)) << pos[j];
  return r;
}

template <int R>
struct RowAddr {
  uint32_t t4;
  uint32_t upos;
  uint32_t tmask;
  uint32_t kpos[R];
  __device__ __forceinline__ const c128 *at(const c128 *p, int k, uint32_t uxor) const {
    const uint32_t u = upos ^ uxor ^ kpos[k];
    const char *b = reinterpret_cast<const char *>(p) + ((uint64_t)(u & ~tmask) << 4);
    return reinterpret_cast<const c128 *>(b + (t4 ^ ((u & tmask) << 4)));
  }
  __device__ __forceinline__ c128 *at(c128 *p, int k, uint32_t uxor) const {
    const uint32_t u = upos ^ uxor ^ kpos[k];
    char *b = reinterpret_cast<char *>(p) + ((uint64_t)(u & ~tmask) << 4);
    return reinterpret_cast<c128 *>(b + (t4 ^ ((u & tmask) << 4)));
  }
};

template <int R, int LOGNT, bool KVAR, bool CPLX, bool PACK>
__device__ __forceinline__ void accum_record(CQuad &Q, double a0, double a1, double a2, double a3,
                                             const c128 (&xv)[R], double (&ar)[R], double (&ai)[R]) {
  if constexpr (PACK && CPLX) {
    const bool fl = Q.nslots != 0u;
    const uint32_t s0 = Q.sign_tile[0] >> LOGNT, s1 = Q.sign_tile[1] >> LOGNT;
    const uint32_t s2 = Q.sign_tile[2] >> LOGNT, s3 = Q.sign_tile[3] >> LOGNT;
#pragma unroll
    for (int k = 0; k < R; ++k) {
      double c0 = a0 + a1, c1 = a2 + a3;
      if constexpr (KVAR) {
        c0 = flip_sign(a0, (uint32_t)__popc(k & s0) & 1u) + flip_sign(a1, (uint32_t)__popc(k & s1) & 1u);
        c1 = flip_sign(a2, (uint32_t)__popc(k & s2) & 1u) + flip_sign(a3, (uint32_t)__popc(k & s3) & 1u);
      }
      ar[k] = fma(c0, fl ? xv[k].y : xv[k].x, ar[k]);
      ai[k] = fma(c1, fl ? xv[k].x : xv[k].y, ai[k]);
    }
  } else if constexpr (!KVAR) {
    const double cre = a0 + a1;
#pragma unroll
    for (int k = 0; k < R; ++k) {
      ar[k] = fma(cre, xv[k].x, ar[k]);
      ai[k] = fma(cre, xv[k].y, ai[k]);
    }
    if constexpr (CPLX) {
      const double cim = a2 + a3;
#pragma unroll
      for (int k = 0; k < R; ++k) {
        ar[k] = fma(-cim, xv[k].y, ar[k]);
        ai[k] = fma(cim, xv[k].x, ai[k]);
      }
    }
  } else {
    const uint32_t s0 = Q.sign_tile[0] >> LOGNT, s1 = Q.sign_tile[1] >> LOGNT;
    const uint32_t s2 = Q.sign_tile[2] >> LOGNT, s3 = Q.sign_tile[3] >> LOGNT;
#pragma unroll
    for (int k = 0; k < R; ++k) {
      const double cre = flip_sign(a0, (uint32_t)__popc(k & s0) & 1u) + flip_sign(a1, (uint32_t)__popc(k & s1) & 1u);
      ar[k] = fma(cre, xv[k].x, ar[k]);
      ai[k] = fma(cre, xv[k].y, ai[k]);
      if constexpr (CPLX) {
        const double cim = flip_sign(a2, (uint32_t)__popc(k & s2) & 1u) + flip_sign(a3, (uint32_t)__popc(k & s3) & 1u);
        ar[k] = fma(-cim, xv[k].y, ar[k]);
        ai[k] = fma(cim, xv[k].x, ai[k]);
      }
    }
  }
}

template <int R, int LOGNT, bool KVAR, bool CPLX, bool GATHER, bool K0, bool PACK = false>
__device__ __forceinline__ void apply_records(CQuad *__restrict__ quads, uint32_t b, uint32_t e,
                                              double (&ar)[R], double (&ai)[R], const c128 *tile,
                                              const RowAddr<R> &RA, const c128 *__restrict__ x,
                                              const c128 *__restrict__ xr, uint32_t tid, uint64_t sbase,
                                              uint32_t skw = 0, uint32_t xrx = 0) {
  constexpr uint32_t NT = 1u << LOGNT;
  for (uint32_t qi = b; qi < e; ++qi) {
    CQuad &Q = quads[qi];
    const double a0 = slot_amp(Q, 0, tid, sbase);
    const double a1 = slot_amp(Q, 1, tid, sbase);
    double a2 = 0.0, a3 = 0.0;
    if constexpr (CPLX) {
      a2 = slot_amp(Q, 2, tid, sbase);
      a3 = slot_amp(Q, 3, tid, sbase);
    }
    c128 xv[R];
    if constexpr (GATHER) {
      const bool live = KVAR || (a0 + a1 != 0.0) || (CPLX && (a2 + a3 != 0.0));
      if (!__any(live)) continue;
      const c128 *__restrict__ src = Q.src ? xr : x;
      const uint32_t mloc = Q.mask_loc;
      const uint32_t xm = (skw ? (mloc ^ (((mloc >> skw) & ((1u << (skw - 4)) - 1u)) << 4)) : mloc) ^ (Q.src ? xrx : 0u);
      if (live) {
#pragma unroll
        for (int k = 0; k < R; ++k) xv[k] = *RA.at(src, k, xm);
      } else {
#pragma unroll
        for (int k = 0; k < R; ++k) xv[k] = make_double2(0.0, 0.0);
      }
    } else if constexpr (K0) {
      const c128 *p = tile + (tid ^ Q.mask_tile);
#pragma unroll
      for (int k = 0; k < R; ++k) xv[k] = p[k * NT];
    } else {
      const uint32_t mt = Q.mask_tile;
      const uint32_t p_lo = tid ^ (mt & (NT - 1u));
      const uint32_t mk = mt >> LOGNT;
#pragma unroll
      for (int k = 0; k < R; ++k) xv[k] = tile[p_lo + (((uint32_t)k ^ mk) << LOGNT)];
    }
    accum_record<R, LOGNT, KVAR, CPLX, PACK>(Q, a0, a1, a2, a3, xv, ar, ai);
  }
}

typedef const __attribute__((address_space(4))) DevTab CTab;

constexpr uint32_t TABB = 32;
constexpr uint32_t TABL_ENTRIES = TABB << MAXTABBITS;

template <int R, int LOGNT, bool GATHER>
__device__ __forceinline__ void apply_tabs(CTab *__restrict__ tabs, const c128 *__restrict__ vals, uint32_t b, uint32_t e,
                                           double (&ar)[R], double (&ai)[R], const c128 *tile, const RowAddr<R> &RA,
                                           const c128 *__restrict__ x, const c128 *__restrict__ xr, uint32_t tid,
                                           uint64_t sbase, uint32_t skw, uint32_t xrx, c128 *tabl) {
  constexpr uint32_t NT = 1u << LOGNT;
  c128 xv[R];
  bool fresh = true;
  for (uint32_t b0 = b; b0 < e; b0 += TABB) {
  const uint32_t b1 = (b0 + TABB < e) ? b0 + TABB : e;
  const uint32_t f0 = tabs[b0].first, f1 = tabs[b1 - 1].first + (1u << tabs[b1 - 1].nbits);
  __syncthreads();
  for (uint32_t i = tid; i < f1 - f0; i += NT) tabl[i] = vals[f0 + i];
  __syncthreads();
  for (uint32_t qi = b0; qi < b1; ++qi) {
    CTab &T = tabs[qi];
    if (fresh) {
      if constexpr (GATHER) {
        const c128 *__restrict__ src = T.src ? xr : x;
        const uint32_t mloc = T.mask_loc;
        const uint32_t xm = (skw ? (mloc ^ (((mloc >> skw) & ((1u << (skw - 4)) - 1u)) << 4)) : mloc) ^ (T.src ? xrx : 0u);
#pragma unroll
        for (int k = 0; k < R; ++k) xv[k] = *RA.at(src, k, xm);
      } else {
        const uint32_t mt = T.mask_tile;
        const uint32_t p_lo = tid ^ (mt & (NT - 1u));
        const uint32_t mk = mt >> LOGNT;
#pragma unroll
        for (int k = 0; k < R; ++k) xv[k] = tile[p_lo + (((uint32_t)k ^ mk) << LOGNT)];
      }
    }
    const uint32_t tp = T.tpos, tw = T.twid, ep = T.epos, ew = T.ewid;
    uint32_t it = 0, is = 0;
#pragma unroll
    for (int q = 0; q < MAXTABBITS; ++q) {
      it |= __builtin_amdgcn_ubfe(tid, (tp >> (8 * q)) & 0xffu, (tw >> (8 * q)) & 0xffu) << q;
      is |= ((uint32_t)(sbase >> ((ep >> (8 * q)) & 0xffu)) & ((ew >> (8 * q)) & 0xffu)) << q;
    }
    it |= is;
    const c128 *tv = tabl + (T.first - f0);
    const uint32_t psign = ((uint32_t)(__popc(tid & T.z_tile) + __popcll(sbase & T.z_ext)) & 1u) << 31;
    const uint32_t ks = T.ksign;
    const uint64_t ikp = T.ik;
    if (T.flags & 1u) {
#pragma unroll
      for (int k = 0; k < R; ++k) {
        const c128 cf = tv[it | ((uint32_t)(ikp >> (4 * k)) & 0xfu)];
        const uint32_t sg = psign ^ (((ks >> k) & 1u) << 31);
        const double cr = __hiloint2double(__double2hiint(cf.x) ^ (int)sg, __double2loint(cf.x));
        const double ci = __hiloint2double(__double2hiint(cf.y) ^ (int)sg, __double2loint(cf.y));
        ar[k] = fma(cr, xv[k].x, ar[k]);
        ar[k] = fma(-ci, xv[k].y, ar[k]);
        ai[k] = fma(cr, xv[k].y, ai[k]);
        ai[k] = fma(ci, xv[k].x, ai[k]);
      }
    } else {
      const c128 c0 = tv[it];
      const double c0r = __hiloint2double(__double2hiint(c0.x) ^ (int)psign, __double2loint(c0.x));
      const double c0i = __hiloint2double(__double2hiint(c0.y) ^ (int)psign, __double2loint(c0.y));
      if (ks == 0u) {
#pragma unroll
        for (int k = 0; k < R; ++k) {
          ar[k] = fma(c0r, xv[k].x, ar[k]);
          ar[k] = fma(-c0i, xv[k].y, ar[k]);
          ai[k] = fma(c0r, xv[k].y, ai[k]);
          ai[k] = fma(c0i, xv[k].x, ai[k]);
        }
      } else
#pragma unroll
      for (int k = 0; k < R; ++k) {
        const uint32_t sg = ((ks >> k) & 1u) << 31;
        const double cr = __hiloint2double(__double2hiint(c0r) ^ (int)sg, __double2loint(c0r));
        const double ci = __hiloint2double(__double2hiint(c0i) ^ (int)sg, __double2loint(c0i));
        ar[k] = fma(cr, xv[k].x, ar[k]);
        ar[k] = fma(-ci, xv[k].y, ar[k]);
        ai[k] = fma(cr, xv[k].y, ai[k]);
        ai[k] = fma(ci, xv[k].x, ai[k]);
      }
    }
    fresh = (T.flags & 2u) != 0u;
  }
  }
}

#ifndef DNM_WAVES_4ROWS
#define DNM_WAVES_4ROWS 8
#endif
constexpr int tile_waves_per_simd(int B, int LOGR, bool TAB = false) {
  if (TAB) {
    int nt = 1 << (B - LOGR);
    int blocks = (160 * 1024) / (16 << B);
    if (blocks < 1) blocks = 1;
    int w = blocks * nt / 256;
    const int cap = LOGR <= 2 ? 8 : 4;
    return w < 1 ? 1 : (w > cap ? cap : w);
  }
  int nt = 1 << (B - LOGR);
  int blocks = (160 * 1024) / (16 << B);
  if (blocks < 1) blocks = 1;
  int w = blocks * nt / 256;
  const int cap = LOGR <= 2 ? DNM_WAVES_4ROWS : 4;
  return w < 1 ? 1 : (w > cap ? cap : w);
}

template <int B, int LOGR, bool GLDS, int GV, bool PACK = false, bool TAB = false>
__global__ void __launch_bounds__(1 << (B - LOGR), tile_waves_per_simd(B, LOGR, TAB))
tile_pass_kernel(const DevPass P, const c128 *__restrict__ x, c128 *__restrict__ y,
                 const c128 *__restrict__ xr) {
  constexpr int R = 1 << LOGR;
  constexpr int LOGNT = B - LOGR;
  constexpr uint32_t NT = 1u << LOGNT;
  extern __shared__ __attribute__((aligned(16))) unsigned char smem[];
  c128 *tile = reinterpret_cast<c128 *>(smem);

  const uint32_t tid = threadIdx.x;
  DNM_PH(0, 0);
  const uint32_t base = deposit<MAXBSEG>(blockIdx.x + P.block_offset, P.nbseg, P.bseg_off, P.bseg_len, P.bseg_pos);
  const uint32_t dep_t = deposit<MAXSEG>(tid, P.nseg, P.seg_off, P.seg_len, P.seg_pos);
  const uint64_t sbase = P.sign_base | (uint64_t)base;

  const uint32_t skw = (uint32_t)P.swz_shift;
  auto lay = [skw](uint32_t v) -> uint32_t { return skw ? (v ^ (((v >> skw) & ((1u << (skw - 4)) - 1u)) << 4)) : v; };
  RowAddr<R> RA;
  RA.t4 = lay(dep_t) << 4;
  RA.upos = lay(base);
  RA.tmask = P.pos_tmask;
#pragma unroll
  for (int k = 0; k < R; ++k) RA.kpos[k] = lay(deposit<MAXSEG>((uint32_t)k << LOGNT, P.nseg, P.seg_off, P.seg_len, P.seg_pos));
  const uint32_t yx = P.swz_xor_y;

  DNM_PRIO_MEM();
  if (!P.need_tile) {
  } else if constexpr (GLDS) {
#pragma unroll
    for (int k = 0; k < R; ++k)
      __builtin_amdgcn_global_load_lds((const GLOBAL_AS void *)RA.at(x, k, 0u),
                                       (LDS_AS void *)(tile + (k * NT + (tid & ~63u))), 16, 0, 0);
  } else {
    c128 v[R];
    if (P.cache_policy & 4) {
#pragma unroll
      for (int k = 0; k < R; ++k) v[k] = load_streaming(RA.at(x, k, 0u));
    } else {
#pragma unroll
      for (int k = 0; k < R; ++k) v[k] = *RA.at(x, k, 0u);
    }
#pragma unroll
    for (int k = 0; k < R; ++k) tile[tid + k * NT] = v[k];
  }
  DNM_PH(1, 1);

  double ar[R], ai[R];
  const bool late_y = P.accumulate && (P.cache_policy & 128);
  if (P.accumulate && !late_y) {
    if (P.cache_policy & 2) {
#pragma unroll
      for (int k = 0; k < R; ++k) {
        c128 v = load_streaming(RA.at((const c128 *)y, k, yx));
        ar[k] = v.x;
        ai[k] = v.y;
      }
    } else {
#pragma unroll
      for (int k = 0; k < R; ++k) {
        c128 v = *RA.at((const c128 *)y, k, yx);
        ar[k] = v.x;
        ai[k] = v.y;
      }
    }
  } else if (P.zinit) {
    const c128 *__restrict__ z = (const c128 *)P.zinit;
    const double zs = -P.zscale;
#pragma unroll
    for (int k = 0; k < R; ++k) {
      const c128 v = load_streaming(RA.at(z, k, yx));
      ar[k] = zs * v.x;
      ai[k] = zs * v.y;
    }
    if (P.zinit2) {
      const c128 *__restrict__ z2 = (const c128 *)P.zinit2;
      const double cr = P.z2re, ci = P.z2im;
#pragma unroll
      for (int k = 0; k < R; ++k) {
        const c128 v = load_streaming(RA.at(z2, k, yx));
        ar[k] = fma(cr, v.x, ar[k]);
        ar[k] = fma(-ci, v.y, ar[k]);
        ai[k] = fma(cr, v.y, ai[k]);
        ai[k] = fma(ci, v.x, ai[k]);
      }
    }
  } else {
#pragma unroll
    for (int k = 0; k < R; ++k) ar[k] = ai[k] = 0.0;
  }

  CQuad *__restrict__ quads = (CQuad *)P.quads;

#define DNM_LOOP(LP, KV, CX, GA, KZ) \
  apply_records<R, LOGNT, KV, CX, GA, KZ, PACK>(quads, P.loop[LP], P.loop[LP + 1], ar, ai, tile, RA, x, xr, tid, sbase, skw, P.swz_xor_src)
  if constexpr (GV >= 1) {
    DNM_LOOP(LP_GATHER_REAL, false, false, true, false);
    DNM_LOOP(LP_GATHER_KVAR_REAL, true, false, true, false);
    DNM_LOOP(LP_GATHER_CPLX, false, true, true, false);
    DNM_LOOP(LP_GATHER_KVAR_CPLX, true, true, true, false);
  }
#undef DNM_LOOP
  c128 *tabl = nullptr;
  if constexpr (TAB) {
    __shared__ __attribute__((aligned(16))) unsigned char tabl_mem[TABL_ENTRIES * 16];
    tabl = reinterpret_cast<c128 *>(tabl_mem);
  }
  if constexpr (TAB)
    apply_tabs<R, LOGNT, true>((CTab *)P.tabs, (const c128 *)P.tabvals, P.tab_loop[1], P.tab_loop[2], ar, ai, tile, RA, x, xr,
                               tid, sbase, skw, P.swz_xor_src, tabl);
  DNM_PH(2, 1);

  double dext = 0.0;
  if (P.has_diag) {
    const uint32_t lane = tid & 63u;
    const uint32_t nterm = (P.dext_end - P.dext_begin) * 4u;
    for (uint32_t t0 = 0; t0 < nterm; t0 += 64u) {
      const uint32_t t = t0 + lane;
      double v = 0.0;
      if (t < nterm) {
        CQuad &Q = quads[P.dext_begin + (t >> 2)];
        const uint32_t j = t & 3u;
        const uint32_t p = (uint32_t)__popcll(sbase & Q.sign_ext[j]) & 1u;
        v = flip_sign(Q.coeff[j], p);
      }
      dext += v;
    }
#pragma unroll
    for (int off = 32; off > 0; off >>= 1) dext += __shfl_xor(dext, off, 64);
  }
  double *cg = nullptr;
  if constexpr (TAB) {
    __shared__ double cg_mem[MAXDGROUPS];
    cg = cg_mem;
    if (P.has_diag) {
      const uint32_t lane = tid & 63u, g0 = P.gbucket[0], g1 = P.gbucket[R];
      for (uint32_t g = g0 + (tid >> 6); g < g1; g += (NT >> 6)) {
        const uint32_t q0 = quads[g].mask_loc, nterm = quads[g].src * 4u;
        double v = 0.0;
        for (uint32_t t0 = 0; t0 < nterm; t0 += 64u) {
          const uint32_t t = t0 + lane;
          if (t < nterm) {
            CQuad &Q = quads[q0 + (t >> 2)];
            const uint32_t j = t & 3u;
            v += flip_sign(Q.coeff[j], (uint32_t)__popcll(sbase & Q.sign_ext[j]) & 1u);
          }
        }
#pragma unroll
        for (int off = 32; off > 0; off >>= 1) v += __shfl_xor(v, off, 64);
        if (lane == 0) cg[g - g0] = v;
      }
    }
  }
  auto diag_part2 = [&]() {
  if (P.has_diag) {
    double D[R];
#pragma unroll
    for (int j = 0; j < R; ++j) D[j] = 0.0;
    D[0] = dext;
    double dtab[R];
    if (P.dtile) {
#pragma unroll
      for (int k = 0; k < R; ++k) dtab[k] = P.dtile[tid + k * NT];
    }
#pragma unroll
    for (int j = 0; j < R; ++j)
      for (uint32_t q = P.dbucket[j]; q < P.dbucket[j + 1]; ++q) {
        const uint32_t ns = quads[q].nslots;
        double v = slot_amp(quads[q], 0, tid, sbase);
        if (ns > 1) v += slot_amp(quads[q], 1, tid, sbase);
        if (ns > 2) v += slot_amp(quads[q], 2, tid, sbase);
        if (ns > 3) v += slot_amp(quads[q], 3, tid, sbase);
        D[j] += v;
      }
    if constexpr (TAB) {
      const uint32_t g0 = P.gbucket[0];
#pragma unroll
      for (int j = 0; j < R; ++j)
        for (uint32_t q = P.gbucket[j]; q < P.gbucket[j + 1]; ++q)
          D[j] += flip_sign(cg[q - g0], (uint32_t)__popc(tid & quads[q].sign_tile[0]) & 1u);
    }
#pragma unroll
    for (int h = 1; h < R; h <<= 1) {
#pragma unroll
      for (int i = 0; i < R; ++i) {
        if ((i & h) == 0) {
          double a = D[i], b = D[i | h];
          D[i] = a + b;
          D[i | h] = a - b;
        }
      }
    }
    if (P.dtile) {
#pragma unroll
      for (int k = 0; k < R; ++k) D[k] += dtab[k];
    }
#pragma unroll
    for (int k = 0; k < R; ++k) {
      c128 xs = tile[tid + k * NT];
      ar[k] = fma(D[k], xs.x, ar[k]);
      ai[k] = fma(D[k], xs.y, ai[k]);
    }
  }
  };
  __syncthreads();
  DNM_PRIO_LDS();
  DNM_PH(3, 0);
  diag_part2();

  DNM_PH(4, 0);
#define DNM_LOOP(LP, KV, CX, GA, KZ) \
  apply_records<R, LOGNT, KV, CX, GA, KZ, PACK>(quads, P.loop[LP], P.loop[LP + 1], ar, ai, tile, RA, x, xr, tid, sbase, skw, P.swz_xor_src)
  DNM_LOOP(LP_TILE_REAL_K0, false, false, false, true);
  DNM_LOOP(LP_TILE_REAL, false, false, false, false);
  DNM_LOOP(LP_TILE_CPLX, false, true, false, false);
  DNM_LOOP(LP_TILE_KVAR_REAL, true, false, false, false);
  DNM_LOOP(LP_TILE_KVAR_CPLX, true, true, false, false);
  if constexpr (GV == 0) {
    DNM_LOOP(LP_GATHER_REAL, false, false, true, false);
    DNM_LOOP(LP_GATHER_KVAR_REAL, true, false, true, false);
    DNM_LOOP(LP_GATHER_CPLX, false, true, true, false);
    DNM_LOOP(LP_GATHER_KVAR_CPLX, true, true, true, false);
  }
#undef DNM_LOOP
  if constexpr (TAB)
    apply_tabs<R, LOGNT, false>((CTab *)P.tabs, (const c128 *)P.tabvals, P.tab_loop[0], P.tab_loop[1], ar, ai, tile, RA, x, xr,
                                tid, sbase, skw, P.swz_xor_src, tabl);

  DNM_PH(5, 0);
  DNM_PRIO_MEM();
  if (late_y) {
    c128 w[R];
#pragma unroll
    for (int k = 0; k < R; ++k) w[k] = load_streaming(RA.at((const c128 *)y, k, yx));
#pragma unroll
    for (int k = 0; k < R; ++k) {
      ar[k] += w[k].x;
      ai[k] += w[k].y;
    }
  }
  DNM_PH(6, 1);
  if (P.cache_policy & 64) {
#pragma unroll
    for (int k = 0; k < R; ++k) store_streaming(RA.at(y, k, yx), ar[k], ai[k]);
  } else if (P.cache_policy & 1) {
#pragma unroll
    for (int k = 0; k < R; ++k) store_through(RA.at(y, k, yx), ar[k], ai[k]);
  } else {
#pragma unroll
    for (int k = 0; k < R; ++k) *RA.at(y, k, yx) = make_double2(ar[k], ai[k]);
  }

  DNM_PH(7, 1);
  if (P.dot_out) {
    double dr = 0.0, di = 0.0, dn = 0.0;
#pragma unroll
    for (int k = 0; k < R; ++k) {
      const c128 xs = tile[tid + k * NT];
      dr = fma(xs.x, ar[k], dr);
      dr = fma(xs.y, ai[k], dr);
      di = fma(xs.x, ai[k], di);
      di = fma(-xs.y, ar[k], di);
      dn = fma(ar[k], ar[k], dn);
      dn = fma(ai[k], ai[k], dn);
    }
#pragma unroll
    for (int off = 32; off > 0; off >>= 1) {
      dr += __shfl_xor(dr, off, 64);
      di += __shfl_xor(di, off, 64);
      dn += __shfl_xor(dn, off, 64);
    }
    __shared__ double dred[3 * (NT / 64 > 0 ? NT / 64 : 1)];
    if ((tid & 63u) == 0) {
      dred[3 * (tid >> 6)] = dr;
      dred[3 * (tid >> 6) + 1] = di;
      dred[3 * (tid >> 6) + 2] = dn;
    }
    __syncthreads();
    if (tid == 0) {
      double sr = 0.0, si = 0.0, sn = 0.0;
      for (uint32_t w = 0; w < NT / 64; ++w) {
        sr += dred[3 * w];
        si += dred[3 * w + 1];
        sn += dred[3 * w + 2];
      }
      P.dot_out[3 * (size_t)blockIdx.x] = sr;
      P.dot_out[3 * (size_t)blockIdx.x + 1] = si;
      P.dot_out[3 * (size_t)blockIdx.x + 2] = sn;
    }
  }
}

#ifdef DNM_PHASE_TIMING
}
extern "C" int dnm_debug_phase_buffer(void *buf) {
  unsigned long long *p = (unsigned long long *)buf;
  return hipMemcpyToSymbol(HIP_SYMBOL(dnm::g_phase_buf), &p, sizeof(p)) == hipSuccess ? 0 : 1;
}
namespace dnm {
#endif

template <int B, int LOGR>
static int launch_cfg(const DevPass &P, bool glds, int n_loc, const void *x, void *y,
                      const void *xr, hipStream_t st, unsigned nparts) {
  constexpr int NT = 1 << (B - LOGR);
  static const size_t lds_req = []() {
    const char *e = knob("DNM_LDS_KB");
    return e ? (size_t)atoi(e) * 1024 : (size_t)0;
  }();
  const size_t lds = std::max(((size_t)16 << B), lds_req);
  const unsigned grid = (1u << (n_loc - B)) / nparts;
  const int gv = (P.cache_policy & 32) ? 1 : 0;
  using kern_t = void (*)(const DevPass, const c128 *, c128 *, const c128 *);
  kern_t k = nullptr;
  const bool pack = (P.cache_policy & 256) != 0;
  const bool tab = P.tab_loop[2] > 0 || P.gbucket[MAXR] > P.gbucket[0];
  if (pack) k = tile_pass_kernel<B, LOGR, false, 1, true>;
  else if (tab) k = tile_pass_kernel<B, LOGR, false, 1, false, true>;
  else if (glds) k = tile_pass_kernel<B, LOGR, true, 1>;
  else if (gv == 0) k = tile_pass_kernel<B, LOGR, false, 0>;
  else k = tile_pass_kernel<B, LOGR, false, 1>;
  static size_t attr_done[6] = {0, 0, 0, 0, 0, 0};
  const int slot = pack ? 4 : (tab ? 5 : (glds ? 3 : gv));
  if (attr_done[slot] < lds) {
    DNM_HIP(hipFuncSetAttribute((const void *)k, hipFuncAttributeMaxDynamicSharedMemorySize, (int)lds));
    attr_done[slot] = lds;
  }
  hipLaunchKernelGGL(k, dim3(grid), dim3(NT), lds, st, P, (const c128 *)x, (c128 *)y, (const c128 *)xr);
  DNM_HIP(hipGetLastError());
  return 0;
}

bool tile_config_supported(int B, int logR) {
  switch (B * 16 + logR) {
    case 10 * 16 + 2: case 11 * 16 + 2: case 12 * 16 + 2:
    case 8 * 16 + 2: case 10 * 16 + 3: case 10 * 16 + 4: case 11 * 16 + 3: case 11 * 16 + 4:
    case 12 * 16 + 3: case 12 * 16 + 4: case 13 * 16 + 3: case 13 * 16 + 4:
      return true;
  }
  return false;
}

int launch_tile_pass(const DevPass &P, int B, int logR, bool glds, int n_loc, const void *x,
                     void *y, const void *xr, hipStream_t st, unsigned nparts) {
  DNM_CHECK(n_loc >= B, "tile larger than the local vector");
  switch (B * 16 + logR) {
    case 8 * 16 + 2: return launch_cfg<8, 2>(P, glds, n_loc, x, y, xr, st, nparts);
    case 10 * 16 + 2: return launch_cfg<10, 2>(P, glds, n_loc, x, y, xr, st, nparts);
    case 11 * 16 + 2: return launch_cfg<11, 2>(P, glds, n_loc, x, y, xr, st, nparts);
    case 12 * 16 + 2: return launch_cfg<12, 2>(P, glds, n_loc, x, y, xr, st, nparts);
    case 10 * 16 + 3: return launch_cfg<10, 3>(P, glds, n_loc, x, y, xr, st, nparts);
    case 10 * 16 + 4: return launch_cfg<10, 4>(P, glds, n_loc, x, y, xr, st, nparts);
    case 11 * 16 + 3: return launch_cfg<11, 3>(P, glds, n_loc, x, y, xr, st, nparts);
    case 11 * 16 + 4: return launch_cfg<11, 4>(P, glds, n_loc, x, y, xr, st, nparts);
    case 12 * 16 + 3: return launch_cfg<12, 3>(P, glds, n_loc, x, y, xr, st, nparts);
    case 12 * 16 + 4: return launch_cfg<12, 4>(P, glds, n_loc, x, y, xr, st, nparts);
    case 13 * 16 + 3: return launch_cfg<13, 3>(P, glds, n_loc, x, y, xr, st, nparts);
    case 13 * 16 + 4: return launch_cfg<13, 4>(P, glds, n_loc, x, y, xr, st, nparts);
  }
  set_error("unsupported tile configuration B=%d logR=%d", B, logR);
  return 1;
}


constexpr int NCK_LDS_MAX = 2 * 1024;

template <int T>
__device__ __forceinline__ SubView stage_sub(const SubView &s, int64_t *lds_tab, int &used) {
  SubView r = s;
  if constexpr (T == DNM_SPIN_CONSERVE) {
    int n = (s.k + 1) * s.ld;
    if (used + n <= NCK_LDS_MAX) {
      for (int i = threadIdx.x; i < n; i += blockDim.x) lds_tab[used + i] = s.nchoosek[i];
      r.nchoosek = lds_tab + used;
      used += n;
    }
  }
  return r;
}

constexpr int GATHER_NT = 256;

__device__ __forceinline__ void mark_column(const ColMark &cm, int64_t col) {
  if (!cm.map) return;
  const int64_t c = (col >> cm.shift) - cm.first;
  const int c32 = (int)c;
  if (__all(c32 == __builtin_amdgcn_readfirstlane(c32))) {
    if ((int)(threadIdx.x & 63) == __ffsll((long long)__ballot(1)) - 1) cm.map[c] = 1;
  } else {
    cm.map[c] = 1;
  }
}

template <int LT, int RT>
__global__ void __launch_bounds__(GATHER_NT)
gather_matvec_kernel(const DevMsc msc, const SubView left_g, const SubView right_g, int64_t M, int64_t row0,
                     int64_t win_start, int xswz, const double *__restrict__ diag, const c128 *__restrict__ x,
                     c128 *__restrict__ y, int64_t *__restrict__ colrange, const ColMark mark) {
  __shared__ int64_t nck[NCK_LDS_MAX];
  int used = 0;
  const SubView left = stage_sub<LT>(left_g, nck, used);
  const SubView right = stage_sub<RT>(right_g, nck, used);
  if (used) __syncthreads();

  const int64_t lrow = (int64_t)blockIdx.x * GATHER_NT + threadIdx.x;
  const bool active = lrow < M;
  if (!active && !colrange) return;
  const int64_t row = row0 + lrow;
  int64_t cmin = INT64_MAX, cmax = INT64_MIN;
  if (active) {
    const int64_t ket = Sub<LT>::i2s(row, left);
    double accr = 0.0, acci = 0.0;
    int m0 = 0;
    if (diag && !colrange) {
      c128 xs = x[vec_pos(row, xswz) - win_start];
      accr = diag[lrow] * xs.x;
      acci = diag[lrow] * xs.y;
      m0 = 1;
    }
    for (int m = m0; m < msc.nmasks; ++m) {
      const int64_t mask = msc.masks[m];
      const int64_t bra = ket ^ mask;
      const int64_t col = Sub<RT>::s2i(bra, right);
      if (col < 0) continue;
      if (colrange) {
        cmin = col < cmin ? col : cmin;
        cmax = col > cmax ? col : cmax;
        mark_column(mark, col);
        continue;
      }
      double cre = 0.0, cim = 0.0;
      for (int64_t t = msc.mask_offsets[m]; t < msc.mask_offsets[m + 1]; ++t) {
        const int64_t sg = msc.signs[t];
        const double c = flip_sign(msc.real_coeffs[t], (uint32_t)__popcll((uint64_t)(bra & sg)) & 1u);
        if (__popcll((uint64_t)(mask & sg)) & 1) cim += c; else cre += c;
      }
      const c128 xv = x[vec_pos(col, xswz) - win_start];
      accr = fma(cre, xv.x, accr);
      acci = fma(cre, xv.y, acci);
      accr = fma(-cim, xv.y, accr);
      acci = fma(cim, xv.x, acci);
    }
    if (!colrange) y[vec_pos(lrow, left.swz)] = make_double2(accr, acci);
  }
  if (colrange) {
    __shared__ int64_t smin[GATHER_NT / 64], smax[GATHER_NT / 64];
    for (int off = 32; off > 0; off >>= 1) {
      const int64_t a = __shfl_xor(cmin, off, 64), b2 = __shfl_xor(cmax, off, 64);
      cmin = a < cmin ? a : cmin;
      cmax = b2 > cmax ? b2 : cmax;
    }
    if ((threadIdx.x & 63) == 0) { smin[threadIdx.x >> 6] = cmin; smax[threadIdx.x >> 6] = cmax; }
    __syncthreads();
    if (threadIdx.x == 0) {
      for (int i = 1; i < GATHER_NT / 64; ++i) {
        cmin = smin[i] < cmin ? smin[i] : cmin;
        cmax = smax[i] > cmax ? smax[i] : cmax;
      }
      colrange[2 * (int64_t)blockIdx.x] = cmin;
      colrange[2 * (int64_t)blockIdx.x + 1] = cmax;
    }
  }
}

constexpr int SC_NT = 256;

template <bool IN_LDS>
__global__ void __launch_bounds__(SC_NT)
sc_matvec_kernel(const DevMsc msc, const ScMask *__restrict__ scm, const ScLow low, const SubView sub_g, int64_t M,
                 int64_t row0, int64_t win_start, const double *__restrict__ diag,
                 const c128 *__restrict__ xw, c128 *__restrict__ y, int64_t *__restrict__ colrange,
                 const ColMark mark) {
  __shared__ int64_t nck[NCK_LDS_MAX];
  const int ld = sub_g.ld, kk = sub_g.k, Lb = sub_g.L;
  const int ntab = (kk + 1) * ld;
  if (IN_LDS) {
    for (int i = threadIdx.x; i < ntab; i += SC_NT) nck[i] = sub_g.nchoosek[i];
    __syncthreads();
  }
#define SC_TAB(i) (IN_LDS ? nck[(i)] : sub_g.nchoosek[(i)])

  const int64_t lrow = (int64_t)blockIdx.x * SC_NT + threadIdx.x;
  const int64_t row = row0 + lrow;
  const c128 *__restrict__ x = xw - win_start;
  int64_t cmin = row, cmax = row;
  const bool active = lrow < M;
  if (!active && !colrange) return;
  if (active) {
  uint64_t ket = 0;
  {
    int64_t idx = row;
    int k = kk;
    for (int n = Lb; n > 16; --n) {
      const int64_t here = (k > n - 1) ? 0 : SC_TAB(k * ld + (n - 1));
      ket <<= 1;
      if (idx >= here) { idx -= here; --k; ket |= 1; }
    }
    const uint64_t lowbits = low.tab[low.off[k] + (int32_t)idx];
    ket = Lb > 16 ? ((ket << 16) | lowbits) : lowbits;
  }
  double accr = 0.0, acci = 0.0;
  int m0 = 0;
  if (diag && !colrange) {
    const c128 xs = x[row];
    const double dg = __builtin_nontemporal_load(diag + lrow);
    accr = dg * xs.x;
    acci = dg * xs.y;
    m0 = 1;
  }
  for (int m = m0; m < msc.nmasks; ++m) {
    if (scm[m].fast) {
// ... 692 lines not shown
```

dynamite_amd/csrc/plan.h:

```cpp
#pragma once

#include <cstdint>
#include <string>
#include <vector>

#include "dnm_common.h"

namespace dnm {

constexpr int MAXSEG = 4;
constexpr int MAXBSEG = 8;
constexpr int MAXSRC = 8;
constexpr int MAXR = 16;

struct RowTerm {
  uint64_t sign;
  double coeff;
  int is_imag;
};

struct RowMask {
  uint64_t mask;
  std::vector<RowTerm> terms;
  bool zero_mask_offdiag = false;
  bool pack_flip = false;
};

struct OpForm {
  bool packed = false;
  int n = 0;
  std::vector<RowMask> masks;
};

struct DevQuad {
  uint32_t mask_tile;
  uint32_t mask_loc;
  uint32_t src;
  uint32_t nslots;
  uint32_t sign_tile[4];
  uint64_t sign_ext[4];
  double coeff[4];
};

constexpr int MAXTABBITS = 4;
struct DevTab {
  uint32_t mask_tile;
  uint32_t mask_loc;
  uint32_t src;
  uint32_t first;
  uint32_t z_tile;
  uint32_t flags;
  uint32_t tpos, twid;
  uint32_t epos, ewid;
  uint64_t z_ext;
  uint64_t ik;
  uint32_t ksign;
  uint32_t nbits;
};

enum {
  LP_TILE_REAL_K0 = 0,
  LP_TILE_REAL,
  LP_TILE_CPLX,
  LP_TILE_KVAR_REAL,
  LP_TILE_KVAR_CPLX,
  LP_GATHER_REAL,
  LP_GATHER_KVAR_REAL,
  LP_GATHER_CPLX,
  LP_GATHER_KVAR_CPLX,
  LP_COUNT
};

struct DevPass {
  int32_t nseg;
  int32_t seg_off[MAXSEG], seg_len[MAXSEG], seg_pos[MAXSEG];
  int32_t nbseg;
  int32_t bseg_off[MAXBSEG], bseg_len[MAXBSEG], bseg_pos[MAXBSEG];
  uint64_t sign_base;
  int32_t accumulate;
  int32_t need_tile;
  int32_t has_diag;
  int32_t cache_policy;
  uint32_t dext_begin, dext_end;
  uint32_t dbucket[MAXR + 1];
  uint32_t loop[LP_COUNT + 1];
  int32_t nquads;
  int32_t n_eff;
  const DevQuad *quads;
  double *dot_out;
  const void *zinit;
  double zscale;
  const void *zinit2;
  double z2re, z2im;
  int32_t tile_bits;
  int32_t log_rows;
  int32_t swz_shift;
  uint32_t swz_xor_y, swz_xor_src;
  uint32_t block_offset;
  uint32_t pos_tmask;
  const double *dtile;
  const DevTab *tabs;
  const double *tabvals;
  uint32_t tab_loop[3];
  uint32_t pad_tab;
  uint32_t gbucket[MAXR + 1];
  uint32_t pad_g;
};
constexpr uint32_t MAXDGROUPS = 64;

struct PassSpec {
  int B = 0;
  int logR = 0;
  int nseg = 0;
  int seg_len[MAXSEG] = {0}, seg_pos[MAXSEG] = {0};
  std::vector<int> tile_masks;
  std::vector<int> gather_masks;
  std::vector<int> gather_src;
  bool has_diag = false;
  bool accumulate = false;
  int partner = -1;
  int n_eff = 0;
  int64_t y_off = 0, src_off = 0;
  uint64_t sign_extra = 0;
  int glen = 0, gpos = 0;
  uint64_t tile_bits() const {
    uint64_t m = 0;
    for (int j = 0; j < nseg; ++j) m |= (((uint64_t)1 << seg_len[j]) - 1) << seg_pos[j];
    return m;
  }
};

struct PlanConfig {
  int B = 12;
  int logR = -1;
  int amin = -1;
  int mode = 2;
  int gbits = -1;
  int Bw = 0, logRw = 0;
  int window_first = -1;
  int gbits_window = -1;
  int cache_policy = 226;
  int max_gather_span = 0;
  int diag_last = -1;
  int swz = 0;
};

struct Plan {
  int n = 0, n_loc = 0;
  int rank = 0, nranks = 1;
  PlanConfig cfg;
  std::vector<PassSpec> local;
  std::vector<PassSpec> remote;
  struct Send { int partner; int64_t offset, count; };
  std::vector<Send> sends;
  bool use_tiled = false;
  std::string describe(const OpForm &op) const;
};

PlanConfig plan_config_from_env();
int make_plan(const OpForm &op, int rank, int nranks, const PlanConfig &cfg, Plan *out);

}
```

include/dynamite_amd.h:

```cpp
#ifndef DYNAMITE_AMD_H
#define DYNAMITE_AMD_H

#include <stddef.h>
#include <stdint.h>

#ifdef __cplusplus
extern "C" {
#endif

const char *dnm_last_error(void);
int dnm_version(void);
int dnm_device_count(int *count);
int dnm_set_device(int device);
int dnm_malloc(void **dptr, size_t bytes);
int dnm_free(void *dptr);
int dnm_memcpy_h2d(void *dst, const void *src, size_t bytes, void *stream);
int dnm_memcpy_d2h(void *dst, const void *src, size_t bytes, void *stream);
int dnm_stream_synchronize(void *stream);

enum { DNM_FULL = 0, DNM_PARITY = 1, DNM_EXPLICIT = 2, DNM_SPIN_CONSERVE = 3 };

typedef struct dnm_subspace {
  int32_t type;
  int64_t L;
  int64_t space;
  int64_t k;
  int64_t ld_nchoosek;
  const int64_t *nchoosek;
  int64_t dim;
  const int64_t *state_map;
  const int64_t *rmap_indices;
  const int64_t *rmap_states;
  int32_t vec_swizzle;
  const int8_t *site_perm;
} dnm_subspace;

int dnm_subspace_dim(const dnm_subspace *s, int64_t *dim);
int dnm_idx_to_state(const dnm_subspace *s, int64_t n, const int64_t *idxs, int64_t *states);
int dnm_state_to_idx(const dnm_subspace *s, int64_t n, const int64_t *states, int64_t *idxs);

int dnm_sc_choose_site_perm(int L, int a, int w, int64_t nmasks, const int64_t *masks, int fix_top, int8_t *site_perm,
                            int32_t *counts);

typedef struct dnm_mat dnm_mat;

enum {
  DNM_MAT_DEFAULT      = 0,
  DNM_MAT_FORCE_GATHER = 1,
  DNM_MAT_USE_GLDS     = 2,
  DNM_MAT_AMIN_SHIFT   = 8,
  DNM_MAT_HOST_ONLY    = 4,
  DNM_MAT_REAL_PACKED  = 16
};

typedef struct dnm_partition {
  int32_t rank;
  int32_t nranks;
} dnm_partition;

int dnm_mat_create(int64_t nmasks, const int64_t *masks, const int64_t *mask_offsets,
                   const int64_t *signs, const double *coeffs,
                   const dnm_subspace *left, const dnm_subspace *right,
                   int xparity, int flags, const dnm_partition *part,
                   dnm_mat **out);
int dnm_check_conserves(int64_t nmasks, const int64_t *masks, const int64_t *mask_offsets,
                        const int64_t *signs, const double *coeffs,
                        const dnm_subspace *left, const dnm_subspace *right,
                        int xparity, int *result, void *stream);
int dnm_reduced_density_matrix(const void *x, const dnm_subspace *sub, int keep_size,
                               const int64_t *keep, void *rho, void *stream);
int dnm_rdm_sector_plan(const dnm_subspace *sub, int keep_size, const int64_t *keep, int xparity_sector,
                        int *nblocks, int32_t *n_of_block, int64_t *dim_of_block, int64_t *traced_of_block,
                        size_t *scratch_bytes_max);
int dnm_rdm_sector_blocks(const void *x, const dnm_subspace *sub, int keep_size, const int64_t *keep,
                          int xparity_sector, int nsel, const int32_t *sel_n, void *const *out_ptrs, void *stream);
int dnm_mat_destroy(dnm_mat *A);
int dnm_mat_sizes(const dnm_mat *A, int64_t *M, int64_t *N, int64_t *m_local, int64_t *n_local);
int dnm_mat_precompute_diagonal(dnm_mat *A, void *stream);
int dnm_mat_get_diagonal(dnm_mat *A, double *diag_host, void *stream);
int dnm_mat_mult(dnm_mat *A, const void *x, void *y, void *stream);
int dnm_mat_norm_inf(dnm_mat *A, double *nrm, void *stream);
int dnm_mat_layouts(const dnm_mat *A, int *left, int *right);
int dnm_mat_is_real_packed(const dnm_mat *A, int *packed);
int dnm_mat_set_norm(dnm_mat *A, double nrm);
int dnm_mat_plan_describe(const dnm_mat *A, char *buf, size_t buflen);
int dnm_mat_plan_launches(const dnm_mat *A, int *n);
int dnm_mat_plan_counts(const dnm_mat *A, int *n_local_passes, int *n_remote_passes, int *tiled,
                        int *B, int *logR, int *n_loc);
int dnm_mat_export_dtile(const dnm_mat *A, int remote, int idx, double *out, int64_t n);
int dnm_mat_export_pass(const dnm_mat *A, int remote, int idx, void *desc_out, size_t desc_bytes,
                        void *quads_out, size_t quad_bytes, int max_quads, int *nquads);
int dnm_mat_export_tabs(const dnm_mat *A, int remote, int idx, void *tabs_out, size_t tab_bytes, int max_tabs, int *ntabs,
                        double *vals_out, int64_t max_vals, int64_t *nvals);

typedef struct {
  int32_t partner;
  int32_t pass_id;
  int64_t offset;
  int64_t count;
} dnm_xfer;
int dnm_mat_exchange_plan(const dnm_mat *A, int *nsend, dnm_xfer *sends ,
                          int *nrecv, dnm_xfer *recvs );
int dnm_mat_mult_dot(dnm_mat *A, const void *x, void *y, double *dot , void *stream);
int dnm_mat_mult_lanczos(dnm_mat *A, const void *x, void *y, const void *z, double b,
                         double *dot , void *stream);
int dnm_mat_mult_sub(dnm_mat *A, const void *x, void *y, const void *z, double b, void *stream);
int dnm_mat_fuses_init(const dnm_mat *A);
int dnm_mat_mult_sub2(dnm_mat *A, const void *x, void *y, const void *z, double b, const void *z2,
                      double c_re, double c_im, void *stream);
int dnm_mat_mult_local(dnm_mat *A, const void *x_local, void *y, void *stream);
int dnm_mat_mult_remote(dnm_mat *A, int32_t recv_index, const void *x_recv,
                        void *y, void *stream);

int dnm_mat_ownership(const dnm_mat *A, int64_t *row0, int64_t *m_local);
int dnm_mat_window_split(const dnm_mat *A, int *supported);
int dnm_mat_mult_local_part(dnm_mat *A, const void *x, void *y, int part, int nparts, void *stream);
int dnm_mat_local_part_bits(const dnm_mat *A, int *top_free_bit, int *gathers);
int dnm_mat_mult_window_local(dnm_mat *A, const void *x_local, void *y_local, void *stream);
int dnm_mat_mult_window_remote(dnm_mat *A, const void *x_window, int64_t win_start, int64_t win_len, void *y_local,
                               void *stream);
int dnm_mat_window_local_rows(dnm_mat *A, int64_t col_lo, int64_t col_hi, int max_ranges, int min_blocks,
                              int64_t *ranges, int *nranges, void *stream);
int dnm_mat_mult_window_rows(dnm_mat *A, const void *x_window, int64_t win_start, int64_t win_len, void *y_local,
                             int64_t r0, int64_t r1, void *stream);
int dnm_mat_column_window(dnm_mat *A, int64_t *cmin, int64_t *cmax, void *stream);
int dnm_mat_column_chunks(dnm_mat *A, int chunk_shift, uint8_t *map, int64_t nchunks, void *stream);
int dnm_mat_column_ranges(dnm_mat *A, int64_t max_ranges, int64_t *ranges, int64_t *nranges);
int dnm_mat_mult_window(dnm_mat *A, const void *x_window, int64_t win_start, int64_t win_len,
                        void *y_local, void *stream);

int dnm_vec_set(void *x, int64_t n, double re, double im, void *stream);
int dnm_vec_copy(const void *x, void *y, int64_t n, void *stream);
int dnm_vec_scale(void *x, int64_t n, double re, double im, void *stream);
int dnm_vec_axpby(void *y, const void *x, int64_t n, double are, double aim,
                  double bre, double bim, void *stream);
int dnm_vec_dot(const void *x, const void *y, int64_t n, double *out, void *stream);
int dnm_vec_norm2(const void *x, int64_t n, double *out, void *stream);
int dnm_vec_set_random(void *x, int64_t n, uint64_t seed, int64_t offset, void *stream);
int dnm_vec_set_random_swz(void *x, int64_t n, uint64_t seed, int64_t offset, int swizzle, void *stream);
int dnm_vec_swizzle_copy(void *dst, const void *src, int64_t n, int swizzle, void *stream);
int dnm_vec_unpack_real(void *dst, const void *src, int64_t n_packed, int swizzle_packed, int swizzle_out, void *stream);
int dnm_vec_layout_unpack_real(const dnm_subspace *s, const dnm_partition *part, void *dst, const void *src, void *stream);
int dnm_vec_layout_size(const dnm_subspace *s, int64_t *n);
int dnm_vec_layout_partition(const dnm_subspace *s, int nranks, int rank, int64_t *istart, int64_t *ilen,
                             int64_t *nstart, int64_t *nlen);
int dnm_vec_layout_blocks(const dnm_subspace *s, int64_t max, int64_t *T, int64_t *ibase, int64_t *count);
int dnm_vec_layout_copy(const dnm_subspace *s, const dnm_partition *part, void *dst, const void *src, int to_internal,
                        void *stream);
int dnm_vec_layout_copy_f64(const dnm_subspace *s, const dnm_partition *part, double *dst, const double *src,
                            int to_internal, void *stream);
int dnm_vec_layout_zero_padding(const dnm_subspace *s, const dnm_partition *part, void *x, void *stream);
int dnm_vec_layout_positions(const dnm_subspace *s, const dnm_partition *part, int64_t n, const int64_t *idx,
                             int64_t *pos, void *stream);
int dnm_vec_layout_positions_host(const dnm_subspace *s, const dnm_partition *part, int64_t n, const int64_t *idx,
                                  int64_t *pos);
int dnm_vec_layout_set_random(const dnm_subspace *s, const dnm_partition *part, void *x, uint64_t seed, void *stream);
int dnm_vec_mdot(const void *V, int64_t ldv, int nv, const void *w, int64_t n,
                 double *h_host, void *stream);
int dnm_vec_maxpy(void *w, const void *V, int64_t ldv, int nv, int64_t n,
                  const double *c_host, void *stream);
int dnm_vec_basis_update(void *V, int64_t ldv, int nin, int nout, int64_t n,
                         const double *S_host, void *stream);

typedef struct dnm_hooks {
  void *ctx;
  int (*mult)(void *ctx, const void *x, void *y);
  int (*allreduce_sum)(void *ctx, double *buf, int n);
  int (*allreduce_max)(void *ctx, double *buf, int n);
} dnm_hooks;

enum {
  DNM_CONVERGED_TOL = 1,
  DNM_CONVERGED_ITS = 2,
  DNM_DIVERGED_ITS = -1,
  DNM_DIVERGED_BREAKDOWN = -2,
  DNM_DIVERGED_SYMMETRY_LOST = -3
};

typedef struct dnm_solver_stats {
  int32_t reason;
  int32_t its;
  int32_t matvecs;
  int32_t nconv;
  double  err_est;
} dnm_solver_stats;

int dnm_expm_multiply(dnm_mat *A, const void *x, void *y, int64_t n_local,
                      double scale_re, double scale_im, double tol, int ncv,
                      int max_its, size_t work_limit_bytes, const dnm_hooks *hooks,
                      dnm_solver_stats *stats, void *stream);

int dnm_expm_chebyshev(dnm_mat *A, const void *x, void *y, int64_t n_local, double t, double tol,
                       const dnm_hooks *hooks, dnm_solver_stats *stats, void *stream);

int dnm_release_workspace(void);
int dnm_workspace_bytes(size_t *bytes);
int dnm_workspace_reserve(size_t bytes, void *stream);

typedef struct dnm_comm dnm_comm;
int dnm_comm_unique_id(void *id128);
int dnm_comm_create(const void *id128, int rank, int nranks, dnm_comm **out);
int dnm_comm_destroy(dnm_comm *c);
int dnm_comm_prepare(dnm_comm *c, dnm_mat *A, void *stream);
int dnm_comm_forget(dnm_comm *c, dnm_mat *A);
int dnm_comm_loopback(dnm_comm *c, int vrank, int vranks, const void *const *peer_x, dnm_mat *const *peer_mat);
int dnm_comm_allreduce(dnm_comm *c, double *vals, int n, int op);
enum { DNM_PHASE_ALL = 0, DNM_PHASE_EXCHANGE = 1, DNM_PHASE_COMPUTE = 2 };
int dnm_comm_set_phase(dnm_comm *c, int phase);
int dnm_mat_mult_partitioned(dnm_mat *A, dnm_comm *c, const void *x, void *y, void *stream);
enum { DNM_EXCHANGE_AUTO = 0, DNM_EXCHANGE_PARTNER = 1, DNM_EXCHANGE_TRANSPOSE = 2 };
int dnm_mat_set_exchange(dnm_mat *A, int scheme, int *chosen);
int dnm_mat_exchange_parts(const dnm_mat *A, dnm_mat **lo, dnm_mat **hi, int *f);
int dnm_mat_operator(const dnm_mat *A, int64_t *nmasks, int64_t *nterms, int64_t *masks, int64_t *mask_offsets,
                     int64_t *signs, double *coeffs);
int dnm_comm_hooks(dnm_comm *c, dnm_mat *A, void *stream, dnm_hooks *out);

enum { DNM_WHICH_LOWEST = 0, DNM_WHICH_HIGHEST = 1, DNM_WHICH_EXTERIOR = 2,
       DNM_WHICH_TARGET = 3  };

int dnm_eigsolve(dnm_mat *A, int64_t n_local, int nev, int which, double tol,
                 int ncv, int max_its, uint64_t seed, const dnm_hooks *hooks,
                 int nev_max, double *evals, void *evecs,
                 dnm_solver_stats *stats, void *stream);

int dnm_eigsolve_interior(dnm_mat *A, int64_t n_local, int nev, double target, double tol,
                          int ncv, int max_its, uint64_t seed, const dnm_hooks *hooks,
                          int nev_max, double *evals, void *evecs,
                          dnm_solver_stats *stats, void *stream);

int dnm_interior_filter_plan(double emin, double emax, double target, double a, double damping,
                             int *degree, double *c, double *e);

#ifdef __cplusplus
}
#endif
#endif
```

Baseline: 64.20.

## Add specialized flip-flop bond records to the tiled Hamiltonian pass kernel

Detects two-site XX+YY-style bonds whose matrix element is a single real constant on anti-aligned spins, and emits them as compact flip records. A dedicated kernel variant applies them via parity-tested swaps, replacing the generic quad records. It also folds matching ZZ diagonal terms into a constant offset. This is meant to cut per-term record decoding and sign arithmetic in the Heisenberg matvec, at the cost of an extra kernel instantiation and more complex plan construction.

```diff
diff --git a/dynamite_amd/_lib.py b/dynamite_amd/_lib.py
--- a/dynamite_amd/_lib.py
+++ b/dynamite_amd/_lib.py
@@ -71,6 +71,15 @@
                 ("z_tile", C.c_uint32), ("flags", C.c_uint32), ("tpos", C.c_uint32), ("twid", C.c_uint32),
                 ("epos", C.c_uint32), ("ewid", C.c_uint32), ("z_ext", C.c_uint64), ("ik", C.c_uint64),
                 ("ksign", C.c_uint32), ("nbits", C.c_uint32)]
+
+
+class DevFlip(C.Structure):
+    _fields_ = [("mask_tile", C.c_uint32), ("mask_pos", C.c_uint32), ("p0", C.c_uint32), ("p1", C.c_uint32),
+                ("pad", C.c_uint32 * 2), ("c", C.c_double)]
+
+
+FL_COUNT = 4
+FL_NAMES = ["tile_thread", "tile_k", "gather_uniform", "gather_boundary"]
 
 
 class Xfer(C.Structure):
@@ -143,6 +152,10 @@
     "dnm_mat_export_tabs": (C.c_int, [vp, C.c_int, C.c_int, vp, C.c_size_t, C.c_int, C.POINTER(C.c_int), f64p, C.c_int64, i64p]),
     "dnm_mat_export_pass": (C.c_int, [vp, C.c_int, C.c_int, vp, C.c_size_t, vp, C.c_size_t, C.c_int,
                                       C.POINTER(C.c_int)]),
+    "dnm_mat_export_flip": (C.c_int, [vp, C.c_int, C.c_int, vp, C.c_size_t, C.c_int, C.POINTER(C.c_int),
+                                      C.POINTER(C.c_uint32), f64p]),
+    "dnm_mat_export_flip_pass": (C.c_int, [vp, C.c_int, C.c_int, vp, C.c_size_t, vp, C.c_size_t, C.c_int,
+                                           C.POINTER(C.c_int), f64p, C.c_int64, i64p]),
     "dnm_mat_ownership": (C.c_int, [vp, i64p, i64p]),
     "dnm_mat_column_window": (C.c_int, [vp, i64p, i64p, vp]),
     "dnm_mat_column_chunks": (C.c_int, [vp, C.c_int, C.POINTER(C.c_uint8), C.c_int64, vp]),
diff --git a/dynamite_amd/csrc/kernels.h b/dynamite_amd/csrc/kernels.h
--- a/dynamite_amd/csrc/kernels.h
+++ b/dynamite_amd/csrc/kernels.h
@@ -18,7 +18,8 @@
 bool tile_config_supported(int B, int logR);
 
 int launch_tile_pass(const DevPass &P, int B, int logR, bool glds, int n_loc,
-                     const void *x, void *y, const void *xr, hipStream_t st, unsigned nparts = 1);
+                     const void *x, void *y, const void *xr, hipStream_t st, unsigned nparts = 1,
+                     const DevFlipPass *F = nullptr);
 
 struct ColMark {
   uint8_t *map = nullptr;
diff --git a/dynamite_amd/csrc/mat.cpp b/dynamite_amd/csrc/mat.cpp
--- a/dynamite_amd/csrc/mat.cpp
+++ b/dynamite_amd/csrc/mat.cpp
@@ -251,111 +251,45 @@
   return nq >= 2 && zs->size() * 45 < nq * 76;
 }
 
-static int build_pass(const dnm_mat &A, const PassSpec &ps, PassOnDevice *out) {
+static const RowMask *diagonal_mask(const OpForm &op) {
+  const RowMask *dm = nullptr;
+  for (const RowMask &m : op.masks) if (m.mask == 0 && !m.zero_mask_offdiag) dm = &m;
+  return dm;
+}
+
+static FlipBond flip_classify(const RowMask &m) {
+  FlipBond fb;
+  if (__builtin_popcountll(m.mask) != 2 || m.zero_mask_offdiag || m.pack_flip) return fb;
+  fb.b0 = __builtin_ctzll(m.mask);
+  fb.b1 = 63 - __builtin_clzll(m.mask);
+  double f[4] = {0.0, 0.0, 0.0, 0.0};
+  for (const RowTerm &t : m.terms) {
+    if (t.is_imag || (t.sign & ~m.mask)) return fb;
+    for (int v = 0; v < 4; ++v) {
+      const int par = ((v & 1) && ((t.sign >> fb.b0) & 1)) ^ ((v & 2) && ((t.sign >> fb.b1) & 1));
+      f[v] += par ? -t.coeff : t.coeff;
+    }
+  }
+  if (f[0] != 0.0 || f[3] != 0.0 || f[1] != f[2] || f[1] == 0.0) return fb;
+  fb.c = f[1];
+  fb.ok = true;
+  return fb;
+}
+
+struct PassTabs {
+  std::vector<DevTab> tile, gather;
+  std::vector<double> vals;
+};
+
+static int emit_records(const dnm_mat &A, const PassSpec &ps, int logR, DevPass &d, std::vector<DevQuad> &quads,
+                        std::vector<double> &h_dtile, PassTabs &T, const std::vector<RowTerm> *dterms,
+                        const std::vector<char> &skip) {
   const OpForm &op = A.op;
-  const Plan &pl = A.plan;
-  const int B = ps.B;
-  int logR = ps.logR ? ps.logR : pl.cfg.logR;
-  {
-    std::vector<uint64_t> zs;
-    bool any = false;
-    for (int idx : ps.tile_masks) any = any || table_form(op, op.masks[idx], &zs);
-    for (int idx : ps.gather_masks) any = any || table_form(op, op.masks[idx], &zs);
-    int want = 3;
-    if (const char *e = knob("DNM_TAB_LOG_ROWS")) want = atoi(e);
-    if (any && want > logR && tile_config_supported(B, want)) logR = want;
-  }
-  {
-    auto top_thread_pos = [&](int lr) {
-      int c = 0, top = -1;
-      for (int j = 0; j < ps.nseg; ++j)
-        for (int i = 0; i < ps.seg_len[j]; ++i, ++c)
-          if (c < B - lr) top = std::max(top, ps.seg_pos[j] + i);
-      return top;
-    };
-    while (top_thread_pos(logR) >= 28 && tile_config_supported(B, logR + 1)) ++logR;
-  }
-  const int lognt = B - logR, R = 1 << logR;
-  const int n_eff = ps.n_eff ? ps.n_eff : pl.n_loc;
+  const int B = ps.B, lognt = B - logR, R = 1 << logR;
+  const int n_eff = ps.n_eff ? ps.n_eff : A.plan.n_loc;
   const uint64_t tb = ps.tile_bits();
-  DevPass &d = out->desc;
-  memset(&d, 0, sizeof(d));
-  d.nseg = ps.nseg;
-  int off = 0;
-  for (int j = 0; j < ps.nseg; ++j) {
-    d.seg_off[j] = off;
-    d.seg_len[j] = ps.seg_len[j];
-    d.seg_pos[j] = ps.seg_pos[j];
-    off += ps.seg_len[j];
-  }
-  DNM_CHECK(off == B, "internal: tile segments do not add up to B");
-  {
-    std::vector<int> order;
-    uint64_t gb = ps.glen ? ((((uint64_t)1 << ps.glen) - 1) << ps.gpos) : 0;
-    std::vector<int> rest;
-    for (int pos = 0; pos < n_eff; ++pos)
-      if (!((tb >> pos) & 1) && !((gb >> pos) & 1)) rest.push_back(pos);
-    size_t nsel = ps.glen ? std::min<size_t>(3, rest.size()) : 0;
-    for (size_t i = 0; i < nsel; ++i) order.push_back(rest[i]);
-    for (int pos = ps.gpos; pos < ps.gpos + ps.glen; ++pos) order.push_back(pos);
-    for (size_t i = nsel; i < rest.size(); ++i) order.push_back(rest[i]);
-    if (const char *e = knob("DNM_ORDER_WINDOW")) {
-      if (ps.nseg > 1 && ps.partner < 0) {
-        std::vector<int> o;
-        for (const char *q = e; *q;) {
-          o.push_back(atoi(q));
-          while (*q && *q != ',') ++q;
-          if (*q == ',') ++q;
-        }
-        std::vector<int> a = o, b2 = order;
-        std::sort(a.begin(), a.end());
-        std::sort(b2.begin(), b2.end());
-        DNM_CHECK(a == b2, "DNM_ORDER_WINDOW is not a permutation of the block bits");
-        order = o;
-      }
-    }
-    DNM_CHECK((int)order.size() == n_eff - B, "internal: block bits do not add up");
-    int nb = 0;
-    for (size_t i = 0; i < order.size();) {
-      size_t j = i + 1;
-      while (j < order.size() && order[j] == order[j - 1] + 1) ++j;
-      DNM_CHECK(nb < MAXBSEG, "internal: too many block segments");
-      d.bseg_off[nb] = (int32_t)i;
-      d.bseg_len[nb] = (int32_t)(j - i);
-      d.bseg_pos[nb] = order[i];
-      ++nb;
-      i = j;
-    }
-    d.nbseg = nb;
-  }
-  d.sign_base = ((uint64_t)pl.rank << pl.n_loc) | ps.sign_extra;
-  d.n_eff = n_eff;
-  d.tile_bits = B;
-  d.log_rows = logR;
-  DNM_CHECK(tile_config_supported(B, logR), "unsupported tile configuration B=%d logR=%d", B, logR);
-  d.accumulate = ps.accumulate ? 1 : 0;
-  d.has_diag = 0;
-  d.cache_policy = pl.cfg.cache_policy | (op.packed ? 256 : 0);
-  {
-    const int S = pl.cfg.swz;
-    DNM_CHECK(S == 0 || (S >= 5 && S <= 24), "swizzle shift %d out of range", S);
-    d.swz_shift = S;
-    auto sw = [S](uint64_t v) -> uint32_t {
-      return S ? (uint32_t)(((v >> S) & (((uint64_t)1 << (S - 4)) - 1)) << 4) : 0u;
-    };
-    d.swz_xor_y = sw((uint64_t)ps.y_off);
-    d.swz_xor_src = sw((uint64_t)ps.src_off);
-    uint64_t tm = 0;
-    int c = 0;
-    for (int j = 0; j < ps.nseg; ++j)
-      for (int i = 0; i < ps.seg_len[j]; ++i, ++c)
-        if (c < lognt) tm |= ((uint64_t)1 << (ps.seg_pos[j] + i)) | sw((uint64_t)1 << (ps.seg_pos[j] + i));
-    DNM_CHECK((tm >> 28) == 0, "internal: thread bits of the tile above bit 27 (tile %llx, %d rows per thread)",
-              (unsigned long long)tb, R);
-    d.pos_tmask = (uint32_t)tm;
-  }
-
-  std::vector<DevQuad> quads;
+  std::vector<DevTab> &tabs_tile = T.tile, &tabs_gather = T.gather;
+  std::vector<double> &tabvals = T.vals;
   auto empty_quad = [&]() {
     DevQuad q;
     memset(&q, 0, sizeof(q));
@@ -378,26 +312,24 @@
   };
 
   if (ps.has_diag) {
-    const RowMask *dm = nullptr;
-    for (const RowMask &m : op.masks) if (m.mask == 0 && !m.zero_mask_offdiag) dm = &m;
-    if (dm) {
+    if (dterms) {
       d.has_diag = 1;
       std::vector<RowTerm> lst;
-      for (const RowTerm &t : dm->terms)
+      for (const RowTerm &t : *dterms)
         if (compress_to_tile(t.sign & tb, ps) == 0) lst.push_back(t);
       d.dext_begin = (uint32_t)quads.size();
       push_diag_list(lst);
       d.dext_end = (uint32_t)quads.size();
       const char *dte = knob("DNM_DIAG_TABLE");
       const bool use_table = !(dte && dte[0] == '0') && B <= 13;
-      if (use_table) out->h_dtile.assign((size_t)1 << B, 0.0);
+      if (use_table) h_dtile.assign((size_t)1 << B, 0.0);
       std::vector<std::pair<uint32_t, std::vector<RowTerm>>> groups;
       {
         const char *dge = knob("DNM_DIAG_GROUPS");
         const bool grouping = !(dge && dge[0] == '0') && !op.packed && !(A.flags & DNM_MAT_USE_GLDS);
         std::vector<std::pair<uint32_t, std::vector<RowTerm>>> all;
         if (grouping)
-          for (const RowTerm &t : dm->terms) {
+          for (const RowTerm &t : *dterms) {
             const uint32_t st = compress_to_tile(t.sign & tb, ps);
             if (st == 0 || (t.sign & ~tb) == 0) continue;
             auto it = std::find_if(all.begin(), all.end(), [&](const auto &g) { return g.first == st; });
@@ -413,12 +345,12 @@
       };
       for (int j = 0; j < R; ++j) {
         lst.clear();
-        for (const RowTerm &t : dm->terms) {
+        for (const RowTerm &t : *dterms) {
           uint32_t st = compress_to_tile(t.sign & tb, ps);
           if (st == 0 || (int)(st >> lognt) != j) continue;
           if (use_table && (t.sign & ~tb) == 0) {
             for (uint32_t tc = 0; tc < (1u << B); ++tc)
-              out->h_dtile[tc] += (__builtin_popcount(tc & st) & 1) ? -t.coeff : t.coeff;
+              h_dtile[tc] += (__builtin_popcount(tc & st) & 1) ? -t.coeff : t.coeff;
           } else if ((t.sign & ~tb) != 0 && grouped(st)) {
             continue;
           } else {
@@ -455,8 +387,6 @@
 
   struct Rec { int loop; DevQuad q; };
   std::vector<Rec> recs;
-  std::vector<DevTab> tabs_tile, tabs_gather;
-  std::vector<double> tabvals;
   auto push_tabs = [&](const RowMask &m, uint64_t mloc, bool gather, int src) -> bool {
     std::vector<uint64_t> zs;
     if (!table_form(op, m, &zs)) return false;
@@ -544,23 +474,134 @@
     }
     return 0;
   };
-  for (int idx : ps.tile_masks) DNM_TRY(push_mask(idx, false, 0));
+  for (int idx : ps.tile_masks)
+    if (skip.empty() || !skip[idx]) DNM_TRY(push_mask(idx, false, 0));
   for (size_t i = 0; i < ps.gather_masks.size(); ++i)
-    DNM_TRY(push_mask(ps.gather_masks[i], true, ps.gather_src[i]));
+    if (skip.empty() || !skip[ps.gather_masks[i]]) DNM_TRY(push_mask(ps.gather_masks[i], true, ps.gather_src[i]));
   for (int lp = 0; lp < LP_COUNT; ++lp) {
     d.loop[lp] = (uint32_t)quads.size();
     for (const Rec &r : recs) if (r.loop == lp) quads.push_back(r.q);
   }
   d.loop[LP_COUNT] = (uint32_t)quads.size();
-
   d.nquads = (int32_t)quads.size();
+  return 0;
+}
+
+static int build_pass(const dnm_mat &A, const PassSpec &ps, PassOnDevice *out) {
+  const OpForm &op = A.op;
+  const Plan &pl = A.plan;
+  const int B = ps.B;
+  int logR = ps.logR ? ps.logR : pl.cfg.logR;
+  {
+    std::vector<uint64_t> zs;
+    bool any = false;
+    for (int idx : ps.tile_masks) any = any || table_form(op, op.masks[idx], &zs);
+    for (int idx : ps.gather_masks) any = any || table_form(op, op.masks[idx], &zs);
+    int want = 3;
+    if (const char *e = knob("DNM_TAB_LOG_ROWS")) want = atoi(e);
+    if (any && want > logR && tile_config_supported(B, want)) logR = want;
+  }
+  {
+    auto top_thread_pos = [&](int lr) {
+      int c = 0, top = -1;
+      for (int j = 0; j < ps.nseg; ++j)
+        for (int i = 0; i < ps.seg_len[j]; ++i, ++c)
+          if (c < B - lr) top = std::max(top, ps.seg_pos[j] + i);
+      return top;
+    };
+    while (top_thread_pos(logR) >= 28 && tile_config_supported(B, logR + 1)) ++logR;
+  }
+  const int lognt = B - logR, R = 1 << logR;
+  const int n_eff = ps.n_eff ? ps.n_eff : pl.n_loc;
+  const uint64_t tb = ps.tile_bits();
+  DevPass &d = out->desc;
+  memset(&d, 0, sizeof(d));
+  d.nseg = ps.nseg;
+  int off = 0;
+  for (int j = 0; j < ps.nseg; ++j) {
+    d.seg_off[j] = off;
+    d.seg_len[j] = ps.seg_len[j];
+    d.seg_pos[j] = ps.seg_pos[j];
+    off += ps.seg_len[j];
+  }
+  DNM_CHECK(off == B, "internal: tile segments do not add up to B");
+  {
+    std::vector<int> order;
+    uint64_t gb = ps.glen ? ((((uint64_t)1 << ps.glen) - 1) << ps.gpos) : 0;
+    std::vector<int> rest;
+    for (int pos = 0; pos < n_eff; ++pos)
+      if (!((tb >> pos) & 1) && !((gb >> pos) & 1)) rest.push_back(pos);
+    size_t nsel = ps.glen ? std::min<size_t>(3, rest.size()) : 0;
+    for (size_t i = 0; i < nsel; ++i) order.push_back(rest[i]);
+    for (int pos = ps.gpos; pos < ps.gpos + ps.glen; ++pos) order.push_back(pos);
+    for (size_t i = nsel; i < rest.size(); ++i) order.push_back(rest[i]);
+    if (const char *e = knob("DNM_ORDER_WINDOW")) {
+      if (ps.nseg > 1 && ps.partner < 0) {
+        std::vector<int> o;
+        for (const char *q = e; *q;) {
+          o.push_back(atoi(q));
+          while (*q && *q != ',') ++q;
+          if (*q == ',') ++q;
+        }
+        std::vector<int> a = o, b2 = order;
+        std::sort(a.begin(), a.end());
+        std::sort(b2.begin(), b2.end());
+        DNM_CHECK(a == b2, "DNM_ORDER_WINDOW is not a permutation of the block bits");
+        order = o;
+      }
+    }
+    DNM_CHECK((int)order.size() == n_eff - B, "internal: block bits do not add up");
+    int nb = 0;
+    for (size_t i = 0; i < order.size();) {
+      size_t j = i + 1;
+      while (j < order.size() && order[j] == order[j - 1] + 1) ++j;
+      DNM_CHECK(nb < MAXBSEG, "internal: too many block segments");
+      d.bseg_off[nb] = (int32_t)i;
+      d.bseg_len[nb] = (int32_t)(j - i);
+      d.bseg_pos[nb] = order[i];
+      ++nb;
+      i = j;
+    }
+    d.nbseg = nb;
+  }
+  d.sign_base = ((uint64_t)pl.rank << pl.n_loc) | ps.sign_extra;
+  d.n_eff = n_eff;
+  d.tile_bits = B;
+  d.log_rows = logR;
+  DNM_CHECK(tile_config_supported(B, logR), "unsupported tile configuration B=%d logR=%d", B, logR);
+  d.accumulate = ps.accumulate ? 1 : 0;
+  d.has_diag = 0;
+  d.cache_policy = pl.cfg.cache_policy | (op.packed ? 256 : 0);
+  {
+    const int S = pl.cfg.swz;
+    DNM_CHECK(S == 0 || (S >= 5 && S <= 24), "swizzle shift %d out of range", S);
+    d.swz_shift = S;
+    auto sw = [S](uint64_t v) -> uint32_t {
+      return S ? (uint32_t)(((v >> S) & (((uint64_t)1 << (S - 4)) - 1)) << 4) : 0u;
+    };
+    d.swz_xor_y = sw((uint64_t)ps.y_off);
+    d.swz_xor_src = sw((uint64_t)ps.src_off);
+    uint64_t tm = 0;
+    int c = 0;
+    for (int j = 0; j < ps.nseg; ++j)
+      for (int i = 0; i < ps.seg_len[j]; ++i, ++c)
+        if (c < lognt) tm |= ((uint64_t)1 << (ps.seg_pos[j] + i)) | sw((uint64_t)1 << (ps.seg_pos[j] + i));
+    DNM_CHECK((tm >> 28) == 0, "internal: thread bits of the tile above bit 27 (tile %llx, %d rows per thread)",
+              (unsigned long long)tb, R);
+    d.pos_tmask = (uint32_t)tm;
+  }
+
+  PassTabs T;
+  std::vector<DevQuad> quads;
+  const RowMask *dm = diagonal_mask(op);
+  DNM_TRY(emit_records(A, ps, logR, d, quads, out->h_dtile, T, dm ? &dm->terms : nullptr, std::vector<char>()));
   d.need_tile = (d.has_diag || !ps.tile_masks.empty()) ? 1 : 0;
   d.tab_loop[0] = 0;
-  d.tab_loop[1] = (uint32_t)tabs_tile.size();
-  d.tab_loop[2] = (uint32_t)(tabs_tile.size() + tabs_gather.size());
-  out->h_tabs = tabs_tile;
-  out->h_tabs.insert(out->h_tabs.end(), tabs_gather.begin(), tabs_gather.end());
-  out->h_tabvals = tabvals;
+  d.tab_loop[1] = (uint32_t)T.tile.size();
+  d.tab_loop[2] = (uint32_t)(T.tile.size() + T.gather.size());
+  out->h_tabs = T.tile;
+  out->h_tabs.insert(out->h_tabs.end(), T.gather.begin(), T.gather.end());
+  out->h_tabvals = T.vals;
   d.tabs = nullptr;
   d.tabvals = nullptr;
   if (!out->h_tabs.empty() && !A.host_only) {
@@ -584,11 +625,150 @@
   return 0;
 }
 
+static void decide_flip_bonds(dnm_mat *A) {
+  const OpForm &op = A->op;
+  const Plan &pl = A->plan;
+  A->flip_bonds.clear();
+  const char *e = knob("DNM_FLIPFLOP");
+  if ((e && e[0] == '0') || op.packed || !(pl.cfg.cache_policy & 32)) return;
+  const RowMask *dm = diagonal_mask(op);
+  bool diag_pass = false;
+  for (size_t i = 0; i < pl.local.size(); ++i) {
+    const DevPass &d = A->local_passes[i]->desc;
+    if (d.tab_loop[2] > 0 || d.gbucket[MAXR] > d.gbucket[0]) return;
+    diag_pass = diag_pass || d.has_diag;
+  }
+  std::vector<FlipBond> bonds(op.masks.size());
+  bool any = false;
+  for (const PassSpec &ps : pl.local) {
+    for (int idx : ps.tile_masks) {
+      FlipBond fb = flip_classify(op.masks[idx]);
+      const uint64_t pair = op.masks[idx].mask;
+      fb.exch = fb.ok && diag_pass && dm &&
+                std::any_of(dm->terms.begin(), dm->terms.end(), [&](const RowTerm &t) { return t.sign == pair; });
+      fb.ok = fb.exch;
+      bonds[idx] = fb;
+      any = any || fb.ok;
+    }
+    for (size_t i = 0; i < ps.gather_masks.size(); ++i) {
+      if (ps.gather_src[i] != 0) continue;
+      bonds[ps.gather_masks[i]] = flip_classify(op.masks[ps.gather_masks[i]]);
+      any = any || bonds[ps.gather_masks[i]].ok;
+    }
+  }
+  if (any) A->flip_bonds.swap(bonds);
+}
+
+static int build_flip_pass(const dnm_mat &A, const PassSpec &ps, PassOnDevice *out) {
+  const OpForm &op = A.op;
+  const Plan &pl = A.plan;
+  const std::vector<FlipBond> &bonds = A.flip_bonds;
+  if (bonds.empty()) return 0;
+  const DevPass &d = out->desc;
+  const int lognt = d.tile_bits - d.log_rows;
+  const uint64_t tb = ps.tile_bits();
+  std::vector<char> skip(op.masks.size(), 0);
+  std::vector<DevFlip> fl[FL_COUNT];
+  const int S = pl.cfg.swz;
+  auto add_flip = [&](int idx, bool gather) {
+    const FlipBond &fb = bonds[idx];
+    if (!fb.ok) return;
+    DevFlip f;
+    memset(&f, 0, sizeof(f));
+    f.c = fb.c;
+    const uint64_t b0 = (uint64_t)1 << fb.b0, b1 = (uint64_t)1 << fb.b1;
+    int cls;
+    if (!gather) {
+      f.mask_tile = compress_to_tile(b0 | b1, ps);
+      f.p0 = (uint32_t)__builtin_ctz(f.mask_tile);
+      f.p1 = 31u - (uint32_t)__builtin_clz(f.mask_tile);
+      cls = (int)f.p1 < lognt ? FL_TILE_T : FL_TILE_K;
+    } else {
+      const uint64_t mloc = b0 | b1;
+      f.mask_pos = (uint32_t)(S ? (mloc ^ (((mloc >> S) & (((uint64_t)1 << (S - 4)) - 1)) << 4)) : mloc);
+      if (!(tb & mloc)) {
+        f.p0 = (uint32_t)fb.b0;
+        f.p1 = (uint32_t)fb.b1;
+        cls = FL_GATHER_U;
+      } else {
+        const bool low_in = (tb & b0) != 0;
+        f.p0 = (uint32_t)__builtin_ctz(compress_to_tile(low_in ? b0 : b1, ps));
+        f.p1 = (uint32_t)(low_in ? fb.b1 : fb.b0);
+        cls = FL_GATHER_B;
+      }
+    }
+    fl[cls].push_back(f);
+    skip[idx] = 1;
+  };
+  for (int idx : ps.tile_masks) add_flip(idx, false);
+  for (int idx : ps.gather_masks) add_flip(idx, true);
+  const RowMask *dm = diagonal_mask(op);
+  std::vector<RowTerm> dterms;
+  if (dm) dterms = dm->terms;
+  double dconst = 0.0;
+  bool diag_changed = false;
+  if (ps.has_diag)
+    for (size_t idx = 0; idx < bonds.size(); ++idx) {
+      if (!bonds[idx].exch) continue;
+      const double a = 0.5 * bonds[idx].c;
+      const uint64_t pair = op.masks[idx].mask;
+      auto it = std::find_if(dterms.begin(), dterms.end(), [&](const RowTerm &t) { return t.sign == pair; });
+      DNM_CHECK(it != dterms.end(), "internal: an exchange without a ZZ term on its pair");
+      if (it->coeff == a) dterms.erase(it);
+      else it->coeff -= a;
+      dconst -= a;
+      diag_changed = true;
+    }
+  size_t nflip = 0;
+  for (int c = 0; c < FL_COUNT; ++c) nflip += fl[c].size();
+  if (nflip == 0 && !diag_changed) return 0;
+  out->fdesc = d;
+  PassTabs T;
+  DNM_TRY(emit_records(A, ps, d.log_rows, out->fdesc, out->h_fquads, out->h_fdtile, T, dm ? &dterms : nullptr, skip));
+  DNM_CHECK(T.tile.empty() && T.gather.empty() && out->fdesc.gbucket[MAXR] == out->fdesc.gbucket[0],
+            "internal: the flip-flop form of a pass has table records or grouped diagonal terms");
+  DevFlipPass &fp = out->flip;
+  memset(&fp, 0, sizeof(fp));
+  for (int c = 0; c < FL_COUNT; ++c) {
+    fp.loop[c] = (uint32_t)out->h_flips.size();
+    out->h_flips.insert(out->h_flips.end(), fl[c].begin(), fl[c].end());
+  }
+  fp.loop[FL_COUNT] = (uint32_t)out->h_flips.size();
+  if (out->h_flips.empty()) out->h_flips.push_back(DevFlip{});
+  fp.dconst = dconst;
+  out->fdesc.quads = nullptr;
+  out->fdesc.dtile = nullptr;
+  if (!A.host_only) {
+    DNM_TRY(out->flips.upload(out->h_flips.data(), out->h_flips.size() * sizeof(DevFlip)));
+    DNM_TRY(out->fquads.upload(out->h_fquads.data(), out->h_fquads.size() * sizeof(DevQuad)));
+    fp.recs = (const DevFlip *)out->flips.p;
+    out->fdesc.quads = (const DevQuad *)out->fquads.p;
+    if (!out->h_fdtile.empty()) {
+      DNM_TRY(out->fdtile.upload(out->h_fdtile.data(), out->h_fdtile.size() * sizeof(double)));
+      out->fdesc.dtile = (const double *)out->fdtile.p;
+    }
+  }
+  return 0;
+}
+
 static hipStream_t S(void *stream) { return (hipStream_t)stream; }
 
 static int launch_pass(const dnm_mat *A, const PassOnDevice &p, const DevPass &d, const void *x, void *y,
                        const void *xr, hipStream_t st, unsigned nparts = 1) {
-  return launch_tile_pass(d, d.tile_bits, d.log_rows, (A->flags & DNM_MAT_USE_GLDS) != 0, p.n_eff, x, y, xr, st, nparts);
+  const bool glds = (A->flags & DNM_MAT_USE_GLDS) != 0;
+  if (p.h_flips.empty()) return launch_tile_pass(d, d.tile_bits, d.log_rows, glds, p.n_eff, x, y, xr, st, nparts);
+  DevPass f = d;
+  const DevPass &k = p.fdesc;
+  f.quads = k.quads;
+  f.dtile = k.dtile;
+  f.nquads = k.nquads;
+  f.has_diag = k.has_diag;
+  f.dext_begin = k.dext_begin;
+  f.dext_end = k.dext_end;
+  memcpy(f.dbucket, k.dbucket, sizeof(f.dbucket));
+  memcpy(f.gbucket, k.gbucket, sizeof(f.gbucket));
+  memcpy(f.loop, k.loop, sizeof(f.loop));
+  return launch_tile_pass(f, f.tile_bits, f.log_rows, glds, p.n_eff, x, y, xr, st, nparts, &p.flip);
 }
 
 static size_t pass_dot_partials(const dnm_mat *, const PassOnDevice &p) {
@@ -1199,6 +1379,9 @@
         DNM_TRY(build_pass(*A, ps, p.get()));
         A->remote_passes.push_back(std::move(p));
       }
+      decide_flip_bonds(A.get());
+      for (size_t i = 0; i < A->plan.local.size(); ++i)
+        DNM_TRY(build_flip_pass(*A, A->plan.local[i], A->local_passes[i].get()));
     }
   }
   *out = A.release();
@@ -1935,6 +2118,53 @@
   return 0;
 }
 
+int dnm_mat_export_flip(const dnm_mat *A, int remote, int idx, void *flips_out, size_t flip_bytes, int max_flips,
+                        int *nflips, uint32_t *loops_out, double *dconst) {
+  DNM_CHECK(A && nflips, "null argument");
+  const auto &v = remote ? A->remote_passes : A->local_passes;
+  DNM_CHECK(idx >= 0 && idx < (int)v.size(), "pass index out of range");
+  const PassOnDevice &p = *v[idx];
+  if (p.h_flips.empty()) {
+    *nflips = -1;
+    return 0;
+  }
+  *nflips = (int)p.flip.loop[FL_COUNT];
+  if (loops_out) memcpy(loops_out, p.flip.loop, sizeof(p.flip.loop));
+  if (dconst) *dconst = p.flip.dconst;
+  if (flips_out && *nflips > 0) {
+    DNM_CHECK(flip_bytes == sizeof(DevFlip), "DevFlip size mismatch (%zu vs %zu)", flip_bytes, sizeof(DevFlip));
+    DNM_CHECK(max_flips >= *nflips, "record buffer too small");
+    memcpy(flips_out, p.h_flips.data(), (size_t)*nflips * sizeof(DevFlip));
+  }
+  return 0;
+}
+
+int dnm_mat_export_flip_pass(const dnm_mat *A, int remote, int idx, void *desc_out, size_t desc_bytes, void *quads_out,
+                             size_t quad_bytes, int max_quads, int *nquads, double *dtile_out, int64_t max_dtile,
+                             int64_t *ndtile) {
+  DNM_CHECK(A && nquads && ndtile, "null argument");
+  const auto &v = remote ? A->remote_passes : A->local_passes;
+  DNM_CHECK(idx >= 0 && idx < (int)v.size(), "pass index out of range");
+  const PassOnDevice &p = *v[idx];
+  DNM_CHECK(!p.h_flips.empty(), "the pass has no flip-flop form");
+  *nquads = (int)p.h_fquads.size();
+  *ndtile = (int64_t)p.h_fdtile.size();
+  if (desc_out) {
+    DNM_CHECK(desc_bytes == sizeof(DevPass), "DevPass size mismatch (%zu vs %zu)", desc_bytes, sizeof(DevPass));
+    memcpy(desc_out, &p.fdesc, sizeof(DevPass));
+  }
+  if (quads_out && !p.h_fquads.empty()) {
+    DNM_CHECK(quad_bytes == sizeof(DevQuad), "DevQuad size mismatch (%zu vs %zu)", quad_bytes, sizeof(DevQuad));
+    DNM_CHECK(max_quads >= *nquads, "record buffer too small");
+    memcpy(quads_out, p.h_fquads.data(), p.h_fquads.size() * sizeof(DevQuad));
+  }
+  if (dtile_out && !p.h_fdtile.empty()) {
+    DNM_CHECK(max_dtile >= *ndtile, "table buffer too small");
+    memcpy(dtile_out, p.h_fdtile.data(), p.h_fdtile.size() * sizeof(double));
+  }
+  return 0;
+}
+
 int dnm_mat_plan_counts(const dnm_mat *A, int *n_local_passes, int *n_remote_passes, int *tiled,
                         int *B, int *logR, int *n_loc) {
   DNM_CHECK(A, "null matrix");
diff --git a/dynamite_amd/csrc/mat.h b/dynamite_amd/csrc/mat.h
--- a/dynamite_amd/csrc/mat.h
+++ b/dynamite_amd/csrc/mat.h
@@ -39,9 +39,22 @@
   std::vector<DevTab> h_tabs;
   std::vector<double> h_tabvals;
   DevBuf tabs, tabvals;
+  std::vector<DevFlip> h_flips;
+  DevFlipPass flip{};
+  DevPass fdesc{};
+  std::vector<DevQuad> h_fquads;
+  std::vector<double> h_fdtile;
+  DevBuf flips, fquads, fdtile;
   int partner = -1;
   int n_eff = 0;
   int64_t y_off = 0, src_off = 0;
+};
+
+struct FlipBond {
+  bool ok = false;
+  bool exch = false;
+  int b0 = 0, b1 = 0;
+  double c = 0.0;
 };
 
 int rdm_release_scratch();
@@ -69,6 +82,7 @@
   dnm::OpForm op;
   dnm::Plan plan;
   std::vector<std::unique_ptr<dnm::PassOnDevice>> local_passes, remote_passes;
+  std::vector<dnm::FlipBond> flip_bonds;
 
   dnm::DevBuf d_masks, d_offsets, d_signs, d_rcoeffs;
   dnm::DevMsc dmsc{};
diff --git a/dynamite_amd/csrc/matvec_kernels.hip b/dynamite_amd/csrc/matvec_kernels.hip
--- a/dynamite_amd/csrc/matvec_kernels.hip
+++ b/dynamite_amd/csrc/matvec_kernels.hip
@@ -58,6 +58,9 @@
 }
 
 __device__ __forceinline__ double slot_amp(CQuad &q, int j, uint32_t tt, uint64_t sbase) {
+#ifdef DNM_PROBE_UNSIGNED_SLOTS
+  return q.coeff[j];
+#endif
   uint32_t p = (uint32_t)(__popc(tt & q.sign_tile[j]) + __popcll(sbase & q.sign_ext[j])) & 1u;
   return flip_sign(q.coeff[j], p);
 }
@@ -181,6 +184,92 @@
       for (int k = 0; k < R; ++k) xv[k] = tile[p_lo + (((uint32_t)k ^ mk) << LOGNT)];
     }
     accum_record<R, LOGNT, KVAR, CPLX, PACK>(Q, a0, a1, a2, a3, xv, ar, ai);
+  }
+}
+
+typedef const __attribute__((address_space(4))) DevFlip CFlip;
+
+struct FlipRec {
+  uint32_t p0, p1, mt;
+  double c;
+};
+__device__ __forceinline__ FlipRec flip_rec(CFlip &F) { return FlipRec{F.p0, F.p1, F.mask_tile, F.c}; }
+
+template <int R, int LOGNT, bool TBITS>
+__device__ __forceinline__ void flip_read(const FlipRec &F, const c128 *tile, uint32_t tid, c128 (&xv)[R]) {
+  constexpr uint32_t NT = 1u << LOGNT;
+  if constexpr (TBITS) {
+    const uint32_t differ = ((tid >> F.p0) ^ (tid >> F.p1)) & 1u;
+    const c128 *p = tile + (tid ^ (F.mt & (0u - differ)));
+#pragma unroll
+    for (int k = 0; k < R; ++k) xv[k] = p[k * NT];
+  } else {
+#pragma unroll
+    for (int k = 0; k < R; ++k) {
+      const uint32_t tc = tid | ((uint32_t)k << LOGNT);
+      const uint32_t differ = ((tc >> F.p0) ^ (tc >> F.p1)) & 1u;
+      xv[k] = tile[tc ^ (F.mt & (0u - differ))];
+    }
+  }
+}
+
+template <int R>
+__device__ __forceinline__ void flip_fma(double c, const c128 (&xv)[R], double (&ar)[R], double (&ai)[R]) {
+#pragma unroll
+  for (int k = 0; k < R; ++k) {
+    ar[k] = fma(c, xv[k].x, ar[k]);
+    ai[k] = fma(c, xv[k].y, ai[k]);
+  }
+}
+
+template <int R, int LOGNT, bool TBITS>
+__device__ __forceinline__ void flip_tile(CFlip *__restrict__ flips, uint32_t b, uint32_t e, double (&ar)[R],
+                                          double (&ai)[R], const c128 *tile, uint32_t tid) {
+  if (b >= e) return;
+  const uint32_t last = e - 1;
+  auto rec = [&](uint32_t i) { return flip_rec(flips[i < last ? i : last]); };
+  c128 xa[R], xb[R];
+  FlipRec f0 = rec(b), f1 = rec(b + 1);
+  flip_read<R, LOGNT, TBITS>(f0, tile, tid, xa);
+  uint32_t qi = b;
+  for (; qi + 1 < e; qi += 2) {
+    const FlipRec g0 = rec(qi + 2), g1 = rec(qi + 3);
+    flip_read<R, LOGNT, TBITS>(f1, tile, tid, xb);
+    flip_fma<R>(f0.c, xa, ar, ai);
+    flip_read<R, LOGNT, TBITS>(g0, tile, tid, xa);
+    flip_fma<R>(f1.c, xb, ar, ai);
+    f0 = g0;
+    f1 = g1;
+  }
+  if (qi < e) flip_fma<R>(f0.c, xa, ar, ai);
+}
+
+template <int R, int LOGNT>
+__device__ __forceinline__ void flip_gathers(CFlip *__restrict__ flips, uint32_t b, uint32_t m, uint32_t e, double (&ar)[R],
+                                             double (&ai)[R], const RowAddr<R> &RA, const c128 *__restrict__ x,
+                                             uint32_t tid, uint64_t sbase) {
+  for (uint32_t qi = b; qi < m; ++qi) {
+    CFlip &F = flips[qi];
+    if (!((uint32_t)((sbase >> F.p0) ^ (sbase >> F.p1)) & 1u)) continue;
+    const uint32_t xm = F.mask_pos;
+    c128 xv[R];
+#pragma unroll
+    for (int k = 0; k < R; ++k) xv[k] = *RA.at(x, k, xm);
+    flip_fma<R>(F.c, xv, ar, ai);
+  }
+  for (uint32_t qi = m; qi < e; ++qi) {
+    CFlip &F = flips[qi];
+    const uint32_t xm = F.mask_pos;
+    const uint32_t outer = (uint32_t)(sbase >> F.p1) & 1u;
+    const uint32_t p0 = F.p0;
+    c128 xv[R];
+#pragma unroll
+    for (int k = 0; k < R; ++k) {
+      const uint32_t tc = tid | ((uint32_t)k << LOGNT);
+      xv[k] = make_double2(0.0, 0.0);
+      if ((((tc >> p0) & 1u) ^ outer) != 0u) xv[k] = *RA.at(x, k, xm);
+    }
+    flip_fma<R>(F.c, xv, ar, ai);
   }
 }
 
@@ -293,10 +382,9 @@
   return w < 1 ? 1 : (w > cap ? cap : w);
 }
 
-template <int B, int LOGR, bool GLDS, int GV, bool PACK = false, bool TAB = false>
-__global__ void __launch_bounds__(1 << (B - LOGR), tile_waves_per_simd(B, LOGR, TAB))
-tile_pass_kernel(const DevPass P, const c128 *__restrict__ x, c128 *__restrict__ y,
-                 const c128 *__restrict__ xr) {
+template <int B, int LOGR, bool GLDS, int GV, bool PACK, bool TAB, bool FLIP>
+__device__ __forceinline__ void tile_pass_body(const DevPass &P, const c128 *__restrict__ x, c128 *__restrict__ y,
+                                               const c128 *__restrict__ xr, const DevFlipPass &FP) {
   constexpr int R = 1 << LOGR;
   constexpr int LOGNT = B - LOGR;
   constexpr uint32_t NT = 1u << LOGNT;
@@ -395,6 +483,9 @@
     DNM_LOOP(LP_GATHER_KVAR_CPLX, true, true, true, false);
   }
 #undef DNM_LOOP
+  if constexpr (FLIP)
+    flip_gathers<R, LOGNT>((CFlip *)FP.recs, FP.loop[FL_GATHER_U], FP.loop[FL_GATHER_B], FP.loop[FL_GATHER_B + 1], ar, ai, RA,
+                           x, tid, sbase);
   c128 *tabl = nullptr;
   if constexpr (TAB) {
     __shared__ __attribute__((aligned(16))) unsigned char tabl_mem[TABL_ENTRIES * 16];
@@ -452,6 +543,7 @@
 #pragma unroll
     for (int j = 0; j < R; ++j) D[j] = 0.0;
     D[0] = dext;
+    if constexpr (FLIP) D[0] += FP.dconst;
     double dtab[R];
     if (P.dtile) {
 #pragma unroll
@@ -505,6 +597,10 @@
   DNM_PH(4, 0);
 #define DNM_LOOP(LP, KV, CX, GA, KZ) \
   apply_records<R, LOGNT, KV, CX, GA, KZ, PACK>(quads, P.loop[LP], P.loop[LP + 1], ar, ai, tile, RA, x, xr, tid, sbase, skw, P.swz_xor_src)
+  if constexpr (FLIP) {
+    flip_tile<R, LOGNT, true>((CFlip *)FP.recs, FP.loop[FL_TILE_T], FP.loop[FL_TILE_T + 1], ar, ai, tile, tid);
+    flip_tile<R, LOGNT, false>((CFlip *)FP.recs, FP.loop[FL_TILE_K], FP.loop[FL_TILE_K + 1], ar, ai, tile, tid);
+  }
   DNM_LOOP(LP_TILE_REAL_K0, false, false, false, true);
   DNM_LOOP(LP_TILE_REAL, false, false, false, false);
   DNM_LOOP(LP_TILE_CPLX, false, true, false, false);
@@ -585,6 +681,20 @@
   }
 }
 
+template <int B, int LOGR, bool GLDS, int GV, bool PACK = false, bool TAB = false>
+__global__ void __launch_bounds__(1 << (B - LOGR), tile_waves_per_simd(B, LOGR, TAB))
+tile_pass_kernel(const DevPass P, const c128 *__restrict__ x, c128 *__restrict__ y,
+                 const c128 *__restrict__ xr) {
+  tile_pass_body<B, LOGR, GLDS, GV, PACK, TAB, false>(P, x, y, xr, DevFlipPass{});
+}
+
+template <int B, int LOGR, bool GLDS>
+__global__ void __launch_bounds__(1 << (B - LOGR), tile_waves_per_simd(B, LOGR, false))
+tile_pass_flip_kernel(const DevPass P, const DevFlipPass FP, const c128 *__restrict__ x, c128 *__restrict__ y,
+                      const c128 *__restrict__ xr) {
+  tile_pass_body<B, LOGR, GLDS, 1, false, false, true>(P, x, y, xr, FP);
+}
+
 #ifdef DNM_PHASE_TIMING
 }
 extern "C" int dnm_debug_phase_buffer(void *buf) {
@@ -596,7 +706,7 @@
 
 template <int B, int LOGR>
 static int launch_cfg(const DevPass &P, bool glds, int n_loc, const void *x, void *y,
-                      const void *xr, hipStream_t st, unsigned nparts) {
+                      const void *xr, hipStream_t st, unsigned nparts, const DevFlipPass *F) {
   constexpr int NT = 1 << (B - LOGR);
   static const size_t lds_req = []() {
     const char *e = knob("DNM_LDS_KB");
@@ -609,6 +719,19 @@
   kern_t k = nullptr;
   const bool pack = (P.cache_policy & 256) != 0;
   const bool tab = P.tab_loop[2] > 0 || P.gbucket[MAXR] > P.gbucket[0];
+  if (F) {
+    DNM_CHECK(!pack && !tab && gv == 1, "internal: flip-flop records in a pass that cannot run them");
+    using fkern_t = void (*)(const DevPass, const DevFlipPass, const c128 *, c128 *, const c128 *);
+    fkern_t fk = glds ? tile_pass_flip_kernel<B, LOGR, true> : tile_pass_flip_kernel<B, LOGR, false>;
+    static size_t fattr_done[2] = {0, 0};
+    if (fattr_done[glds ? 1 : 0] < lds) {
+      DNM_HIP(hipFuncSetAttribute((const void *)fk, hipFuncAttributeMaxDynamicSharedMemorySize, (int)lds));
+      fattr_done[glds ? 1 : 0] = lds;
+    }
+    hipLaunchKernelGGL(fk, dim3(grid), dim3(NT), lds, st, P, *F, (const c128 *)x, (c128 *)y, (const c128 *)xr);
+    DNM_HIP(hipGetLastError());
+    return 0;
+  }
   if (pack) k = tile_pass_kernel<B, LOGR, false, 1, true>;
   else if (tab) k = tile_pass_kernel<B, LOGR, false, 1, false, true>;
   else if (glds) k = tile_pass_kernel<B, LOGR, true, 1>;
@@ -636,21 +759,21 @@
 }
 
 int launch_tile_pass(const DevPass &P, int B, int logR, bool glds, int n_loc, const void *x,
-                     void *y, const void *xr, hipStream_t st, unsigned nparts) {
+                     void *y, const void *xr, hipStream_t st, unsigned nparts, const DevFlipPass *F) {
   DNM_CHECK(n_loc >= B, "tile larger than the local vector");
   switch (B * 16 + logR) {
-    case 8 * 16 + 2: return launch_cfg<8, 2>(P, glds, n_loc, x, y, xr, st, nparts);
-    case 10 * 16 + 2: return launch_cfg<10, 2>(P, glds, n_loc, x, y, xr, st, nparts);
-    case 11 * 16 + 2: return launch_cfg<11, 2>(P, glds, n_loc, x, y, xr, st, nparts);
-    case 12 * 16 + 2: return launch_cfg<12, 2>(P, glds, n_loc, x, y, xr, st, nparts);
-    case 10 * 16 + 3: return launch_cfg<10, 3>(P, glds, n_loc, x, y, xr, st, nparts);
-    case 10 * 16 + 4: return launch_cfg<10, 4>(P, glds, n_loc, x, y, xr, st, nparts);
-    case 11 * 16 + 3: return launch_cfg<11, 3>(P, glds, n_loc, x, y, xr, st, nparts);
-    case 11 * 16 + 4: return launch_cfg<11, 4>(P, glds, n_loc, x, y, xr, st, nparts);
-    case 12 * 16 + 3: return launch_cfg<12, 3>(P, glds, n_loc, x, y, xr, st, nparts);
-    case 12 * 16 + 4: return launch_cfg<12, 4>(P, glds, n_loc, x, y, xr, st, nparts);
-    case 13 * 16 + 3: return launch_cfg<13, 3>(P, glds, n_loc, x, y, xr, st, nparts);
-    case 13 * 16 + 4: return launch_cfg<13, 4>(P, glds, n_loc, x, y, xr, st, nparts);
+    case 8 * 16 + 2: return launch_cfg<8, 2>(P, glds, n_loc, x, y, xr, st, nparts, F);
+    case 10 * 16 + 2: return launch_cfg<10, 2>(P, glds, n_loc, x, y, xr, st, nparts, F);
+    case 11 * 16 + 2: return launch_cfg<11, 2>(P, glds, n_loc, x, y, xr, st, nparts, F);
+    case 12 * 16 + 2: return launch_cfg<12, 2>(P, glds, n_loc, x, y, xr, st, nparts, F);
+    case 10 * 16 + 3: return launch_cfg<10, 3>(P, glds, n_loc, x, y, xr, st, nparts, F);
+    case 10 * 16 + 4: return launch_cfg<10, 4>(P, glds, n_loc, x, y, xr, st, nparts, F);
+    case 11 * 16 + 3: return launch_cfg<11, 3>(P, glds, n_loc, x, y, xr, st, nparts, F);
+    case 11 * 16 + 4: return launch_cfg<11, 4>(P, glds, n_loc, x, y, xr, st, nparts, F);
+    case 12 * 16 + 3: return launch_cfg<12, 3>(P, glds, n_loc, x, y, xr, st, nparts, F);
+    case 12 * 16 + 4: return launch_cfg<12, 4>(P, glds, n_loc, x, y, xr, st, nparts, F);
+    case 13 * 16 + 3: return launch_cfg<13, 3>(P, glds, n_loc, x, y, xr, st, nparts, F);
+    case 13 * 16 + 4: return launch_cfg<13, 4>(P, glds, n_loc, x, y, xr, st, nparts, F);
   }
   set_error("unsupported tile configuration B=%d logR=%d", B, logR);
   return 1;
diff --git a/dynamite_amd/csrc/plan.h b/dynamite_amd/csrc/plan.h
--- a/dynamite_amd/csrc/plan.h
+++ b/dynamite_amd/csrc/plan.h
@@ -108,6 +108,27 @@
 };
 constexpr uint32_t MAXDGROUPS = 64;
 
+struct DevFlip {
+  uint32_t mask_tile;
+  uint32_t mask_pos;
+  uint32_t p0, p1;
+  uint32_t pad[2];
+  double c;
+};
+enum {
+  FL_TILE_T = 0,
+  FL_TILE_K,
+  FL_GATHER_U,
+  FL_GATHER_B,
+  FL_COUNT
+};
+struct DevFlipPass {
+  const DevFlip *recs;
+  uint32_t loop[FL_COUNT + 1];
+  uint32_t pad;
+  double dconst;
+};
+
 struct PassSpec {
   int B = 0;
   int logR = 0;
diff --git a/include/dynamite_amd.h b/include/dynamite_amd.h
--- a/include/dynamite_amd.h
+++ b/include/dynamite_amd.h
@@ -92,6 +92,11 @@
                         void *quads_out, size_t quad_bytes, int max_quads, int *nquads);
 int dnm_mat_export_tabs(const dnm_mat *A, int remote, int idx, void *tabs_out, size_t tab_bytes, int max_tabs, int *ntabs,
                         double *vals_out, int64_t max_vals, int64_t *nvals);
+int dnm_mat_export_flip(const dnm_mat *A, int remote, int idx, void *flips_out, size_t flip_bytes, int max_flips,
+                        int *nflips, uint32_t *loops_out, double *dconst);
+int dnm_mat_export_flip_pass(const dnm_mat *A, int remote, int idx, void *desc_out, size_t desc_bytes, void *quads_out,
+                             size_t quad_bytes, int max_quads, int *nquads, double *dtile_out, int64_t max_dtile,
+                             int64_t *ndtile);
 
 typedef struct {
   int32_t partner;
```

Measured after the change: 66.89 (median of 6 runs). +4.2%, better.
